# PKU-EPIC/GAPartNet

Hardware: AMD Instinct MI355X
Metric: point-clouds/sec (20k pts, train step) (higher is better)
Workload: dtype f32

## Files before the change

gapartnet_amd/_C.py:

```python
import ctypes
import os
import subprocess

_HERE = os.path.dirname(os.path.abspath(__file__))
SO_PATH = os.path.join(_HERE, "libgpn_hip.so")
CSRC = os.path.join(_HERE, "csrc")

_lib = None

_SIZE_T_FUNCS = (
    "gpn_voxelize_ws_bytes", "gpn_voxelize_scenes_ws_bytes", "gpn_rulebook_subm3_ws_bytes", "gpn_rulebook_down_ws_bytes",
    "gpn_rulebook_down_lists_ws_bytes", "gpn_rulebook_level_counts_ws_bytes", "gpn_spconv_fwd_ws_bytes", "gpn_spconv_fwd_w_ws_bytes", "gpn_net_ws_bytes", "gpn_linear_bwd_ws_bytes", "gpn_ball_query_grid_ws_bytes", "gpn_point_losses_ws_bytes", "gpn_rulebook_tile_order_ws_bytes", "gpn_bn_ws_bytes", "gpn_spconv_wgrad_ws_bytes", "gpn_ccl_ws_bytes", "gpn_nms_ws_bytes", "gpn_pn2_furthest_point_sampling_ws_bytes", "gpn_pose_fit_ws_bytes", "gpn_proposals_revoxelize_ws_bytes", "gpn_proposals_postprocess_ws_bytes", "gpn_backbone_prepare_arena_bytes", "gpn_scene_prepare_ws_bytes",
    "gpn_view_fps_ws_bytes", "gpn_net_forward_bf16_ws_bytes", "gpn_scene_maps_ws_bytes", "gpn_boxes_draw_ws_bytes",
    "gpn_pointmlp_wgrad_ws_bytes",
)


class GpnError(RuntimeError):
    pass


def build(jobs: int = 8) -> str:
    subprocess.check_call(["make", "-C", CSRC, "-s", "-j", str(jobs)])
    return SO_PATH


def lib():
    global _lib
    if _lib is None:
        if not os.path.exists(SO_PATH):
            raise GpnError(
                f"{SO_PATH} is missing: the HIP extension has not been built. Run "
                "`python -c 'import __graft_entry__ as g; g.build()'` (needs hipcc). There is no CPU fallback.")
        import torch
        _lib = ctypes.CDLL(SO_PATH)
        _lib.gpn_last_error.restype = ctypes.c_char_p
        _lib.gpn_entry_point_name.restype = ctypes.c_char_p
        for name in _SIZE_T_FUNCS:
            getattr(_lib, name).restype = ctypes.c_size_t
        vp, i64t, i32t, f32t, st = ctypes.c_void_p, ctypes.c_int64, ctypes.c_int, ctypes.c_float, ctypes.c_size_t
        _lib.gpn_spconv_fwd_w.argtypes = [vp, vp, i32t, i32t, i32t, i32t, vp, i64t, vp, vp, st, vp]
        _lib.gpn_spconv_wgrad.argtypes = [vp, vp, vp, vp, vp, i32t, i64t, i32t, i32t, i32t, vp, vp, st, vp]
        _lib.gpn_bn_fwd_train.argtypes = [vp, vp, vp, vp, i64t, i32t, f32t, f32t, i32t, vp, vp, vp, vp, vp, vp, st, vp]
        _lib.gpn_bn_fwd_eval.argtypes = [vp, vp, vp, vp, vp, vp, i64t, i32t, i32t, vp, vp]
        _lib.gpn_bn_bwd.argtypes = [vp, vp, vp, vp, vp, vp, i64t, i32t, i32t, i32t, vp, vp, vp, vp, vp, st, vp]
        _lib.gpn_gather_rows.argtypes = [vp, vp, i64t, i32t, vp, vp]
        _lib.gpn_scatter_rows_csr.argtypes = [vp, vp, vp, i64t, i32t, vp, vp]
        _lib.gpn_spconv_tiles_min_tiles.argtypes = [i64t]
        _lib.gpn_spconv_tiles_min_tiles.restype = i64t
        _lib.gpn_spconv_direct_split.argtypes = [i64t, i64t]
        _lib.gpn_spconv_msplit.argtypes = [i32t, i32t, i32t]
    return _lib


def check(rc: int, what: str = ""):
    if rc != 0:
        msg = lib().gpn_last_error().decode("utf-8", "replace")
        raise GpnError(f"{what or 'gpn call'} failed (code {rc}): {msg}")


def ptr(t):
    if t is None:
        return ctypes.c_void_p(0)
    return ctypes.c_void_p(t.data_ptr())


def i64(v):
    return ctypes.c_int64(int(v))


def i32(v):
    return ctypes.c_int(int(v))


def f32(v):
    return ctypes.c_float(float(v))


def szt(v):
    return ctypes.c_size_t(int(v))


def host_f32x3(v):
    return (ctypes.c_float * 3)(*[float(x) for x in v])


def host_i32x3(v):
    return (ctypes.c_int32 * 3)(*[int(x) for x in v])
```

gapartnet_amd/csrc/ballquery.hip:

```cpp
#include "gpn_common.h"

#include <rocprim/rocprim.hpp>

namespace {

constexpr int kThreads = 256;
constexpr int kWaves = kThreads / 64;
constexpr int kCap = 256;
constexpr int kMaxCell = 32766;

struct GridHeader {
  unsigned int min_enc[3];
  unsigned int overflow;
};

__device__ __forceinline__ unsigned int enc_float(float f) {
  const unsigned int b = __float_as_uint(f);
  return (b & 0x80000000u) ? ~b : (b | 0x80000000u);
}
__device__ __forceinline__ float dec_float(unsigned int u) {
  return __uint_as_float((u & 0x80000000u) ? (u & 0x7fffffffu) : ~u);
}

__global__ void bq_init_kernel(GridHeader* hdr) {
  hdr->min_enc[0] = hdr->min_enc[1] = hdr->min_enc[2] = 0xffffffffu;
  hdr->overflow = 0u;
}

__global__ __launch_bounds__(kThreads) void bq_min_kernel(const float* __restrict__ points, int64_t Np, GridHeader* hdr) {
  __shared__ unsigned int smin[3];
  if (threadIdx.x < 3) smin[threadIdx.x] = 0xffffffffu;
  __syncthreads();
  unsigned int m[3] = {0xffffffffu, 0xffffffffu, 0xffffffffu};
  for (int64_t j = (int64_t)blockIdx.x * kThreads + threadIdx.x; j < Np; j += (int64_t)gridDim.x * kThreads) {
#pragma unroll
    for (int a = 0; a < 3; ++a) {
      const unsigned int e = enc_float(points[j * 3 + a]);
      m[a] = e < m[a] ? e : m[a];
    }
  }
#pragma unroll
  for (int a = 0; a < 3; ++a) atomicMin(&smin[a], m[a]);
  __syncthreads();
  if (threadIdx.x < 3) atomicMin(&hdr->min_enc[threadIdx.x], smin[threadIdx.x]);
}

__device__ __forceinline__ int cell_of(float x, float origin, float inv_cell) {
  const float c = floorf(__fmul_rn(__fsub_rn(x, origin), inv_cell));
  return (int)fminf(fmaxf(c, -4.0f), 40000.0f) + 1;
}

__device__ __forceinline__ uint64_t pack_key(int seg, int cx, int cy, int cz) {
  return ((uint64_t)(unsigned)seg << 48) | ((uint64_t)(unsigned)cx << 32) | ((uint64_t)(unsigned)cy << 16) | (uint64_t)(unsigned)cz;
}

__global__ __launch_bounds__(kThreads) void bq_keys_kernel(const float* __restrict__ points,
                                                           const int32_t* __restrict__ point_labels,
                                                           const int32_t* __restrict__ batch_offsets, int64_t Np, int64_t S,
                                                           float inv_cell, GridHeader* hdr, uint64_t* __restrict__ keys,
                                                           int32_t* __restrict__ vals) {
  const int64_t j = (int64_t)blockIdx.x * kThreads + threadIdx.x;
  if (j >= Np) return;
  if (point_labels && point_labels[j] < 0) {
    keys[j] = ~0ull;
    vals[j] = (int32_t)j;
    return;
  }
  int64_t lo = 0, hi = S;
  while (hi - lo > 1) {
    const int64_t mid = (lo + hi) >> 1;
    if ((int64_t)batch_offsets[mid] <= j) lo = mid; else hi = mid;
  }
  const int seg = (int)lo;
  const float ox = dec_float(hdr->min_enc[0]), oy = dec_float(hdr->min_enc[1]), oz = dec_float(hdr->min_enc[2]);
  const int cx = cell_of(points[j * 3], ox, inv_cell), cy = cell_of(points[j * 3 + 1], oy, inv_cell),
            cz = cell_of(points[j * 3 + 2], oz, inv_cell);
  if (cx < 1 || cy < 1 || cz < 1 || cx > kMaxCell || cy > kMaxCell || cz > kMaxCell || seg > 65535) hdr->overflow = 1u;
  keys[j] = pack_key(seg & 0xffff, cx & 0x7fff, cy & 0x7fff, cz & 0x7fff);
  vals[j] = (int32_t)j;
}

__global__ __launch_bounds__(kThreads) void bq_records_kernel(const float* __restrict__ points,
                                                              const int32_t* __restrict__ point_labels,
                                                              const int32_t* __restrict__ order, int64_t Np,
                                                              float4* __restrict__ rec) {
  const int64_t j = (int64_t)blockIdx.x * kThreads + threadIdx.x;
  if (j >= Np) return;
  const int32_t o = order[j];
  float4 r;
  r.x = points[(int64_t)o * 3];
  r.y = points[(int64_t)o * 3 + 1];
  r.z = points[(int64_t)o * 3 + 2];
  r.w = __int_as_float(point_labels ? point_labels[o] : 0);
  rec[j] = r;
}

__device__ __forceinline__ bool is_hit(float qx, float qy, float qz, float px, float py, float pz, float r2) {
  const float dx = __fsub_rn(qx, px), dy = __fsub_rn(qy, py), dz = __fsub_rn(qz, pz);
  const float d2 = __fadd_rn(__fadd_rn(__fmul_rn(dx, dx), __fmul_rn(dy, dy)), __fmul_rn(dz, dz));
  return d2 < r2;
}

__global__ __launch_bounds__(kThreads) void bq_query_kernel(
    const float* __restrict__ points, const float* __restrict__ query, const int32_t* __restrict__ batch_indices,
    const int32_t* __restrict__ batch_offsets, const int32_t* __restrict__ point_labels,
    const int32_t* __restrict__ query_labels, int64_t Np, int64_t Q, float r2, float inv_cell, int K,
    const GridHeader* __restrict__ hdr, const uint64_t* __restrict__ keys, const int32_t* __restrict__ order,
    const float4* __restrict__ rec, int32_t* __restrict__ indices, int32_t* __restrict__ count) {
  __shared__ int32_t hits[kWaves][kCap];
  const int lane = threadIdx.x & 63, wave = threadIdx.x >> 6;
  const int64_t q = (int64_t)blockIdx.x * kWaves + wave;
  if (q >= Q) return;
  const float qx = query[q * 3], qy = query[q * 3 + 1], qz = query[q * 3 + 2];
  const int32_t b = batch_indices[q];
  const int32_t lo = batch_offsets[b], hi = batch_offsets[b + 1];
  const bool use_labels = point_labels != nullptr && query_labels != nullptr;
  const int32_t ql = use_labels ? query_labels[q] : 0;
  if (ql < 0) {
    if (lane == 0) count[q] = 0;
    return;
  }
  int32_t* out = indices + q * K;
  const uint64_t lane_lt = (1ull << lane) - 1ull;

  bool fallback = hdr->overflow != 0u || b > 65535;
  int H = 0;
  if (!fallback) {
    const float ox = dec_float(hdr->min_enc[0]), oy = dec_float(hdr->min_enc[1]), oz = dec_float(hdr->min_enc[2]);
    const int cx = cell_of(qx, ox, inv_cell), cy = cell_of(qy, oy, inv_cell), cz = cell_of(qz, oz, inv_cell);
    int32_t bound = 0;
    if (lane < 18) {
      const int t = lane < 9 ? lane : lane - 9;
      const int x = cx + t / 3 - 1, y = cy + t % 3 - 1;
      int z0 = cz - 1, z1 = cz + 1;
      const bool empty = x < 1 || y < 1 || x > kMaxCell || y > kMaxCell || z1 < 1 || z0 > kMaxCell;
      z0 = z0 < 1 ? 1 : z0;
      z1 = z1 > kMaxCell ? kMaxCell : z1;
      if (!empty) {
        const bool upper = lane >= 9;
        const uint64_t key = pack_key(b, x, y, upper ? z1 : z0);
        int64_t l = 0, h = Np;
        while (l < h) {
          const int64_t mid = (l + h) >> 1;
          const uint64_t k = keys[mid];
          if (upper ? (k <= key) : (k < key)) l = mid + 1; else h = mid;
        }
        bound = (int32_t)l;
      }
    }
    int32_t start[9], len[9];
    int total = 0;
#pragma unroll
    for (int t = 0; t < 9; ++t) {
      start[t] = __shfl(bound, t, 64);
      const int32_t e = __shfl(bound, t + 9, 64);
      len[t] = e > start[t] ? e - start[t] : 0;
      total += len[t];
    }
    for (int base = 0; base < total && !fallback; base += 64) {
      int c = base + lane;
      bool hit = false;
      int32_t o = -1;
      if (c < total) {
        int32_t j = 0;
#pragma unroll
        for (int t = 0; t < 9; ++t) {
          if (c >= 0 && c < len[t]) j = start[t] + c;
          c -= len[t];
        }
        const float4 r = rec[j];
        if (!use_labels || __float_as_int(r.w) == ql) {
          if (is_hit(qx, qy, qz, r.x, r.y, r.z, r2)) {
            o = order[j];
            hit = o >= lo && o < hi;
          }
        }
      }
      const uint64_t mask = __builtin_amdgcn_ballot_w64(hit);
      const int pos = H + __popcll(mask & lane_lt);
      if (hit && pos < kCap) hits[wave][pos] = o;
      H += __popcll(mask);
      if (H > kCap) fallback = true;
    }
  }

  if (!fallback) {
    for (int i = lane; i < H; i += 64) {
      const int32_t v = hits[wave][i];
      int rank = 0;
      for (int m = 0; m < H; ++m) rank += hits[wave][m] < v ? 1 : 0;
      if (rank < K) out[rank] = v;
    }
    if (lane == 0) count[q] = H < K ? H : K;
    return;
  }

  int cnt = 0;
  for (int32_t base = lo; base < hi && cnt < K; base += 64) {
    const int32_t j = base + lane;
    bool hit = false;
    if (j < hi && (!use_labels || point_labels[j] == ql))
      hit = is_hit(qx, qy, qz, points[(int64_t)j * 3], points[(int64_t)j * 3 + 1], points[(int64_t)j * 3 + 2], r2);
    const uint64_t mask = __builtin_amdgcn_ballot_w64(hit);
    const int pos = cnt + __popcll(mask & lane_lt);
    if (hit && pos < K) out[pos] = j;
    cnt += __popcll(mask);
  }
  if (lane == 0) count[q] = cnt < K ? cnt : K;
}

struct BqWs {
  GridHeader* hdr;
  uint64_t *keys, *keys_sorted;
  int32_t *vals, *order;
  float4* rec;
  void* prim_tmp;
  size_t prim_bytes, total;
};

BqWs carve(void* ws, size_t ws_bytes, int64_t Np) {
  gpn::WsCarver w(ws, ws_bytes);
  const size_t n = (size_t)(Np > 0 ? Np : 1);
  BqWs o;
  o.hdr = w.take<GridHeader>(1);
  o.keys = w.take<uint64_t>(n);
  o.keys_sorted = w.take<uint64_t>(n);
  o.vals = w.take<int32_t>(n);
  o.order = w.take<int32_t>(n);
  o.rec = w.take<float4>(n);
  o.prim_bytes = 0;
  (void)rocprim::radix_sort_pairs(nullptr, o.prim_bytes, (const uint64_t*)nullptr, (uint64_t*)nullptr,
                                  (const int32_t*)nullptr, (int32_t*)nullptr, n, 0, 64, (hipStream_t) nullptr);
  o.prim_tmp = w.take<char>(o.prim_bytes);
  o.total = w.used;
  return o;
}

}

extern "C" size_t gpn_ball_query_grid_ws_bytes(int64_t Np) { return carve(nullptr, 0, Np).total; }

extern "C" int gpn_ball_query_grid(const float* points, const float* query, const int32_t* batch_indices,
                                   const int32_t* batch_offsets, const int32_t* point_labels,
                                   const int32_t* query_labels, int64_t Np, int64_t Q, int64_t S, float radius, int K,
                                   int32_t* indices, int32_t* count, void* ws, size_t ws_bytes, gpn_stream_t stream_) {
  hipStream_t stream = (hipStream_t)stream_;
  const bool pad = !(K & GPN_BQ_NO_PAD);
  K &= ~GPN_BQ_NO_PAD;
  GPN_CHECK_ARG(Q >= 0 && Np >= 0 && S >= 0 && K >= 1 && radius > 0.f);
  if (Q == 0) return GPN_OK;
  GPN_CHECK_ARG(points && query && batch_indices && batch_offsets && indices && count);
  GPN_CHECK_ARG(Np < (int64_t)0x7fffffff && Q * (int64_t)K < ((int64_t)1 << 40));
  BqWs o = carve(ws, ws_bytes, Np);
  if (!ws || ws_bytes < o.total) {
    gpn::set_error("gpn_ball_query_grid: workspace too small (%zu needed, %zu given)", o.total, ws_bytes);
    return GPN_ERR_WS;
  }
  const float r2 = radius * radius;
  const float inv_cell = 1.0f / (1.05f * radius);
  gpn::ProfScope prof(GPN_K_BALL_QUERY, stream, 0.0, 12.0 * (double)Np + 4.0 * (double)Q * K);
  if (pad) GPN_CHECK_HIP(hipMemsetAsync(indices, 0xff, sizeof(int32_t) * (size_t)Q * K, stream));
  hipLaunchKernelGGL(bq_init_kernel, dim3(1), dim3(1), 0, stream, o.hdr);
  GPN_CHECK_LAUNCH();
  if (Np > 0) {
    const int pgrid = (int)gpn::cdiv(Np, kThreads);
    hipLaunchKernelGGL(bq_min_kernel, dim3(pgrid < 256 ? pgrid : 256), dim3(kThreads), 0, stream, points, Np, o.hdr);
    GPN_CHECK_LAUNCH();
    hipLaunchKernelGGL(bq_keys_kernel, dim3(pgrid), dim3(kThreads), 0, stream, points, point_labels, batch_offsets, Np, S,
                       inv_cell, o.hdr, o.keys, o.vals);
    GPN_CHECK_LAUNCH();
    size_t tmp = o.prim_bytes;
    GPN_CHECK_HIP(rocprim::radix_sort_pairs(o.prim_tmp, tmp, o.keys, o.keys_sorted, o.vals, o.order, (size_t)Np, 0, 64,
                                            stream));
    hipLaunchKernelGGL(bq_records_kernel, dim3(pgrid), dim3(kThreads), 0, stream, points, point_labels, o.order, Np,
                       o.rec);
    GPN_CHECK_LAUNCH();
  }
  hipLaunchKernelGGL(bq_query_kernel, dim3((unsigned)gpn::cdiv(Q, kWaves)), dim3(kThreads), 0, stream, points, query,
                     batch_indices, batch_offsets, point_labels, query_labels, Np, Q, r2, inv_cell, K, o.hdr,
                     o.keys_sorted, o.order, o.rec, indices, count);
  GPN_CHECK_LAUNCH();
  return GPN_OK;
}
```

gapartnet_amd/csrc/cluster.hip:

```cpp
#include "gpn_common.h"

namespace {

constexpr int kThreads = 256;

__global__ __launch_bounds__(kThreads) void ball_query_kernel(
    const float* __restrict__ points, const float* __restrict__ query, const int32_t* __restrict__ batch_indices,
    const int32_t* __restrict__ batch_offsets, const int32_t* __restrict__ point_labels,
    const int32_t* __restrict__ query_labels, int64_t Q, float r2, int K, int32_t* __restrict__ indices,
    int32_t* __restrict__ count) {
  __shared__ float4 tile[kThreads];
  __shared__ int32_t range_lo, range_hi;
  const int64_t q = (int64_t)blockIdx.x * kThreads + threadIdx.x;
  const bool active = q < Q;
  float qx = 0.f, qy = 0.f, qz = 0.f;
  int32_t lo = 0x7fffffff, hi = 0, ql = 0;
  if (active) {
    qx = query[q * 3]; qy = query[q * 3 + 1]; qz = query[q * 3 + 2];
    const int32_t b = batch_indices[q];
    lo = batch_offsets[b];
    hi = batch_offsets[b + 1];
    if (query_labels) ql = query_labels[q];
  }
  if (threadIdx.x == 0) { range_lo = 0x7fffffff; range_hi = 0; }
  __syncthreads();
  if (active && lo < hi) { atomicMin(&range_lo, lo); atomicMax(&range_hi, hi); }
  __syncthreads();
  const int32_t blo = range_lo, bhi = range_hi;
  const bool use_labels = point_labels != nullptr && query_labels != nullptr;
  int cnt = 0;
  int32_t* out = indices + q * K;
  for (int32_t base = blo; base < bhi; base += kThreads) {
    const int32_t j = base + threadIdx.x;
    if (j < bhi) {
      float4 rec;
      rec.x = points[(int64_t)j * 3]; rec.y = points[(int64_t)j * 3 + 1]; rec.z = points[(int64_t)j * 3 + 2];
      rec.w = __int_as_float(use_labels ? point_labels[j] : 0);
      tile[threadIdx.x] = rec;
    }
    __syncthreads();
    const int32_t n_here = (bhi - base < kThreads) ? (bhi - base) : kThreads;
    if (active && cnt < K && base < hi && base + n_here > lo) {
      int32_t t0 = lo > base ? lo - base : 0;
      int32_t t1 = hi - base < n_here ? hi - base : n_here;
      for (int32_t t = t0; t < t1 && cnt < K; ++t) {
        const float4 rec = tile[t];
        if (use_labels && __float_as_int(rec.w) != ql) continue;
        const float dx = __fsub_rn(qx, rec.x), dy = __fsub_rn(qy, rec.y), dz = __fsub_rn(qz, rec.z);
        const float d2 = __fadd_rn(__fadd_rn(__fmul_rn(dx, dx), __fmul_rn(dy, dy)), __fmul_rn(dz, dz));
        if (d2 < r2) out[cnt++] = base + t;
      }
    }
    const int done = (!active) || cnt >= K || (base + kThreads >= hi);
    if (__syncthreads_and(done)) break;
  }
  if (active) count[q] = cnt;
}

__device__ __forceinline__ int32_t uf_load(const int32_t* p) {
  return __hip_atomic_load(p, __ATOMIC_RELAXED, __HIP_MEMORY_SCOPE_WORKGROUP);
}
__device__ __forceinline__ int32_t uf_find(int32_t* parent, int32_t x) {
  int32_t p = uf_load(parent + x);
  while (p != x) {
    const int32_t gp = uf_load(parent + p);
    if (gp != p) __hip_atomic_store(parent + x, gp, __ATOMIC_RELAXED, __HIP_MEMORY_SCOPE_WORKGROUP);
    x = p;
    p = gp;
  }
  return x;
}
__device__ __forceinline__ void uf_union(int32_t* parent, int32_t ra, int32_t rb) {
  while (ra != rb) {
    if (ra < rb) { const int32_t tmp = ra; ra = rb; rb = tmp; }
    int32_t old = __hip_atomic_load(parent + ra, __ATOMIC_RELAXED, __HIP_MEMORY_SCOPE_AGENT);
    if (old == ra) {
      old = atomicCAS(parent + ra, ra, rb);
      if (old == ra) break;
    }
    ra = uf_find(parent, old);
    rb = uf_find(parent, rb);
  }
}

__global__ void ccl_init_kernel(const int32_t* __restrict__ begin_end, const int32_t* __restrict__ edges, int64_t Q,
                                int32_t* parent) {
  const int64_t v = ((int64_t)blockIdx.x * blockDim.x + threadIdx.x) >> 6;
  const int lane = threadIdx.x & 63;
  if (v >= Q) return;
  const int32_t b = begin_end[2 * v], e = begin_end[2 * v + 1];
  int32_t m = (int32_t)v;
  for (int32_t t = b + lane; t < e; t += 64) {
    const int32_t u = edges[t];
    if (u >= 0 && u < m) m = u;
  }
#pragma unroll
  for (int off = 32; off >= 1; off >>= 1) {
    const int32_t o = __shfl_xor(m, off, 64);
    m = o < m ? o : m;
  }
  if (lane == 0) parent[v] = m;
}

__global__ void ccl_compress_kernel(int32_t* parent, int64_t Q) {
  const int64_t i = (int64_t)blockIdx.x * blockDim.x + threadIdx.x;
  if (i >= Q) return;
  const int32_t r = uf_find(parent, (int32_t)i);
  if (r != (int32_t)i) __hip_atomic_store(parent + i, r, __ATOMIC_RELAXED, __HIP_MEMORY_SCOPE_WORKGROUP);
}

__global__ void ccl_hook_kernel(const int32_t* __restrict__ begin_end, const int32_t* __restrict__ edges,
                                int64_t Q, int32_t* parent) {
  const int64_t v = ((int64_t)blockIdx.x * blockDim.x + threadIdx.x) >> 6;
  const int lane = threadIdx.x & 63;
  if (v >= Q) return;
  const int32_t b = begin_end[2 * v], e = begin_end[2 * v + 1];
  for (int32_t t0 = b; t0 < e; t0 += 64) {
    const int32_t t = t0 + lane;
    int32_t u = t < e ? edges[t] : (int32_t)v;
    if (u < 0 || u >= Q) u = (int32_t)v;
    const int32_t pv = uf_load(parent + v);
    const bool same = uf_load(parent + u) == pv;
    if (__builtin_amdgcn_ballot_w64(!same) == 0) continue;
    const int32_t r = uf_find(parent, same ? (int32_t)v : u);
    int32_t m = r;
#pragma unroll
    for (int off = 32; off >= 1; off >>= 1) {
      const int32_t o = __shfl_xor(m, off, 64);
      m = o < m ? o : m;
    }
    uint64_t todo = __builtin_amdgcn_ballot_w64(r != m);
    while (todo) {
      const int leader = __builtin_ctzll(todo);
      const int32_t rl = __builtin_amdgcn_readlane(r, leader);
      if (lane == leader) uf_union(parent, rl, m);
      todo &= ~__builtin_amdgcn_ballot_w64(r == rl);
    }
  }
}

__global__ void ccl_flatten_kernel(int32_t* parent, int64_t Q, int32_t* __restrict__ labels,
                                   int32_t* __restrict__ is_root) {
  int64_t i = (int64_t)blockIdx.x * blockDim.x + threadIdx.x;
  if (i >= Q) return;
  const int32_t r = uf_find(parent, (int32_t)i);
  labels[i] = r;
  if (is_root) is_root[i] = (r == (int32_t)i) ? 1 : 0;
}

__global__ void ccl_rank_kernel(const int32_t* __restrict__ is_root, int64_t Q, int32_t* __restrict__ rank) {
  __shared__ int32_t sums[1024];
  __shared__ int32_t carry;
  if (threadIdx.x == 0) carry = 0;
  __syncthreads();
  for (int64_t base = 0; base < Q; base += 1024) {
    const int64_t i = base + threadIdx.x;
    const int32_t v = i < Q ? is_root[i] : 0;
    sums[threadIdx.x] = v;
    __syncthreads();
    for (int off = 1; off < 1024; off <<= 1) {
      int32_t t = threadIdx.x >= off ? sums[threadIdx.x - off] : 0;
      __syncthreads();
      sums[threadIdx.x] += t;
      __syncthreads();
    }
    if (i < Q) rank[i] = carry + sums[threadIdx.x] - v;
    __syncthreads();
    if (threadIdx.x == 1023) carry += sums[1023];
    __syncthreads();
  }
}
__global__ void ccl_relabel_kernel(int32_t* __restrict__ labels, const int32_t* __restrict__ rank, int64_t Q) {
  int64_t i = (int64_t)blockIdx.x * blockDim.x + threadIdx.x;
  if (i < Q) labels[i] = rank[labels[i]];
}

template <int MODE>
__global__ void segmented_reduce_kernel(const float* __restrict__ values, const int32_t* __restrict__ begin,
                                        const int32_t* __restrict__ end, int64_t P, int C,
                                        float* __restrict__ out) {
  int64_t t = (int64_t)blockIdx.x * blockDim.x + threadIdx.x;
  if (t >= P * C) return;
  const int64_t p = t / C;
  const int c = (int)(t - p * C);
  const int32_t b = begin[p], e = end[p];
  float acc = 0.f;
  for (int32_t r = b; r < e; ++r) {
    const float v = values[(int64_t)r * C + c];
    if (r == b) acc = v;
    else if (MODE == 0) acc = __fadd_rn(acc, v);
    else if (MODE == 1) acc = v < acc ? v : acc;
    else acc = v > acc ? v : acc;
  }
  out[t] = acc;
}

__global__ void segmented_maxpool_fwd_kernel(const float* __restrict__ values, const int32_t* __restrict__ begin,
                                             const int32_t* __restrict__ end, int64_t P, int C,
                                             float* __restrict__ pooled, int32_t* __restrict__ argmax) {
  int64_t t = (int64_t)blockIdx.x * blockDim.x + threadIdx.x;
  if (t >= P * C) return;
  const int64_t p = t / C;
  const int c = (int)(t - p * C);
  float best = 0.f;
  int32_t bi = -1;
  for (int32_t r = begin[p]; r < end[p]; ++r) {
    const float v = values[(int64_t)r * C + c];
    if (bi < 0 || v > best) { best = v; bi = r; }
  }
  pooled[t] = best;
  argmax[t] = bi;
}

__global__ __launch_bounds__(256) void segmented_maxpool_fwd_wg_kernel(const float* __restrict__ values,
                                                                       const int32_t* __restrict__ begin,
                                                                       const int32_t* __restrict__ end, int C,
                                                                       float* __restrict__ pooled, int32_t* __restrict__ argmax,
                                                                       int64_t P, const int64_t* __restrict__ p_dev) {
  __shared__ float sv[256];
  __shared__ int32_t si[256];
  P = gpn::live_rows(p_dev, P);
  const int R = 256 / C;
  const int c = threadIdx.x % C, rl = threadIdx.x / C;
  for (int64_t p = blockIdx.x; p < P; p += gridDim.x) {
  float best = 0.f;
  int32_t bi = -1;
  if (rl < R) {
    const int32_t b = begin[p], e = end[p];
    for (int32_t r = b + rl; r < e; r += R) {
      const float v = values[(int64_t)r * C + c];
      if (bi < 0 || v > best) { best = v; bi = r; }
    }
  }
  sv[threadIdx.x] = best;
  si[threadIdx.x] = bi;
  __syncthreads();
  if (threadIdx.x < C) {
    for (int q = 1; q < R; ++q) {
      const float v = sv[q * C + c];
      const int32_t i = si[q * C + c];
      if (i >= 0 && (bi < 0 || v > best || (v == best && i < bi))) { best = v; bi = i; }
    }
    pooled[p * C + c] = best;
    argmax[p * C + c] = bi;
  }
  __syncthreads();
  }
}

__global__ void segmented_maxpool_bwd_kernel(const float* __restrict__ dpooled, const int32_t* __restrict__ argmax,
                                             int64_t P, int C, float* __restrict__ dvalues, const int64_t* __restrict__ p_dev) {
  P = gpn::live_rows(p_dev, P);
  for (int64_t t = (int64_t)blockIdx.x * blockDim.x + threadIdx.x; t < P * C; t += (int64_t)gridDim.x * blockDim.x) {
    const int c = (int)(t % C);
    const int32_t r = argmax[t];
    if (r >= 0) dvalues[(int64_t)r * C + c] = dpooled[t];
  }
}
__global__ void zero_rows_kernel(float* __restrict__ p, int64_t rows, int C, const int64_t* __restrict__ m_dev) {
  const int64_t total = gpn::live_rows(m_dev, rows) * C;
  for (int64_t t = (int64_t)blockIdx.x * blockDim.x + threadIdx.x; t < total; t += (int64_t)gridDim.x * blockDim.x) p[t] = 0.f;
}

__global__ void instance_iou_kernel(const int32_t* __restrict__ proposal_offsets,
                                    const int32_t* __restrict__ instance_labels,
                                    const int32_t* __restrict__ batch_indices,
                                    const int32_t* __restrict__ npi, int64_t P, int I, float* __restrict__ ious,
                                    const int64_t* __restrict__ p_dev) {
  extern __shared__ int32_t hist[];
  P = gpn::live_rows(p_dev, P);
  for (int64_t p = blockIdx.x; p < P; p += gridDim.x) {
  const int32_t b0 = proposal_offsets[p], b1 = proposal_offsets[p + 1];
  for (int k = threadIdx.x; k < I; k += blockDim.x) hist[k] = 0;
  __syncthreads();
  for (int32_t m = b0 + threadIdx.x; m < b1; m += blockDim.x) {
    const int32_t l = instance_labels[m];
    if (l >= 0 && l < I) atomicAdd(&hist[l], 1);
  }
  __syncthreads();
  const int32_t b = b1 > b0 ? batch_indices[b0] : 0;
  for (int k = threadIdx.x; k < I; k += blockDim.x) {
    const int32_t n = npi[(int64_t)b * I + k];
    const int32_t uni = (b1 - b0) + n - hist[k];
    ious[p * I + k] = (n > 0 && uni > 0) ? __fdiv_rn((float)hist[k], (float)uni) : 0.f;
  }
  __syncthreads();
  }
}

__global__ void nms_mask_kernel(const float* __restrict__ ious, const int32_t* __restrict__ order, int64_t P,
                                int64_t W, float thr, unsigned long long* __restrict__ mask) {
  int64_t t = (int64_t)blockIdx.x * blockDim.x + threadIdx.x;
  if (t >= P * W) return;
  const int64_t a = t / W, w = t - a * W;
  const int32_t i = order[a];
  unsigned long long bits = 0;
  for (int bpos = 0; bpos < 64; ++bpos) {
    const int64_t bb = w * 64 + bpos;
    if (bb < P && bb > a && ious[(int64_t)i * P + order[bb]] > thr) bits |= 1ull << bpos;
  }
  mask[t] = bits;
}

__global__ void nms_scan_kernel(const unsigned long long* __restrict__ mask, const int32_t* __restrict__ order,
                                int64_t P, int64_t W, int32_t* __restrict__ keep, int32_t* __restrict__ num_keep) {
  extern __shared__ unsigned long long removed[];
  for (int64_t w = threadIdx.x; w < W; w += blockDim.x) removed[w] = 0;
  __syncthreads();
  int32_t n = 0;
  for (int64_t a = 0; a < P; ++a) {
    const bool dead = (removed[a >> 6] >> (a & 63)) & 1ull;
    __syncthreads();
    if (!dead) {
      if (threadIdx.x == 0) keep[n] = order[a];
      ++n;
      for (int64_t w = threadIdx.x; w < W; w += blockDim.x) removed[w] |= mask[a * W + w];
    }
    __syncthreads();
  }
  if (threadIdx.x == 0) num_keep[0] = n;
}

}

extern "C" int gpn_ball_query(const float* points, const float* query, const int32_t* batch_indices,
                              const int32_t* batch_offsets, const int32_t* point_labels,
                              const int32_t* query_labels, int64_t Np, int64_t Q, int64_t S, float radius, int K,
                              int32_t* indices, int32_t* count, gpn_stream_t stream_) {
  hipStream_t stream = (hipStream_t)stream_;
  GPN_CHECK_ARG(Q >= 0 && Np >= 0 && S >= 0 && K >= 1);
  if (Q == 0) return GPN_OK;
  GPN_CHECK_ARG(points && query && batch_indices && batch_offsets && indices && count);
  GPN_CHECK_ARG(Np < (int64_t)0x7fffffff);
  const float r2 = radius * radius;
  gpn::ProfScope prof(GPN_K_BALL_QUERY, stream, 0.0, 12.0 * (double)Np + 4.0 * (double)Q * K);
  GPN_CHECK_HIP(hipMemsetAsync(indices, 0xff, sizeof(int32_t) * (size_t)Q * K, stream));
  hipLaunchKernelGGL(ball_query_kernel, dim3((int)gpn::cdiv(Q, kThreads)), dim3(kThreads), 0, stream, points,
                     query, batch_indices, batch_offsets, point_labels, query_labels, Q, r2, K, indices, count);
  GPN_CHECK_LAUNCH();
  return GPN_OK;
}

extern "C" size_t gpn_ccl_ws_bytes(int64_t Q) {
  gpn::WsCarver w(nullptr, 0);
  size_t q = (size_t)(Q > 0 ? Q : 1);
  w.take<int32_t>(q);
  w.take<int32_t>(q);
  w.take<int32_t>(q);
  return w.used;
}

extern "C" int gpn_ccl(const int32_t* begin_end, const int32_t* edges, int64_t Q, int64_t E, int compacted,
                       int32_t* labels, void* ws, size_t ws_bytes, gpn_stream_t stream_) {
  hipStream_t stream = (hipStream_t)stream_;
  GPN_CHECK_ARG(Q >= 0 && E >= 0);
  if (Q == 0) return GPN_OK;
  GPN_CHECK_ARG(begin_end && labels && (edges || E == 0));
  GPN_CHECK_ARG(Q < (int64_t)0x7fffffff / 64);
  gpn::WsCarver w(ws, ws_bytes);
  int32_t* parent = w.take<int32_t>((size_t)Q);
  int32_t* is_root = w.take<int32_t>((size_t)Q);
  int32_t* rank = w.take<int32_t>((size_t)Q);
  GPN_CHECK_WS(w);
  const int grid = (int)gpn::cdiv(Q, kThreads);
  gpn::ProfScope prof(GPN_K_CCL, stream, 0.0, 4.0 * ((double)E + 2.0 * (double)Q) + 4.0 * (double)Q);
  hipLaunchKernelGGL(ccl_init_kernel, dim3((int)gpn::cdiv(Q * 64, kThreads)), dim3(kThreads), 0, stream, begin_end, edges,
                     Q, parent);
  GPN_CHECK_LAUNCH();
  hipLaunchKernelGGL(ccl_compress_kernel, dim3(grid), dim3(kThreads), 0, stream, parent, Q);
  GPN_CHECK_LAUNCH();
  hipLaunchKernelGGL(ccl_hook_kernel, dim3((int)gpn::cdiv(Q * 64, kThreads)), dim3(kThreads), 0, stream,
                     begin_end, edges, Q, parent);
  GPN_CHECK_LAUNCH();
  hipLaunchKernelGGL(ccl_flatten_kernel, dim3(grid), dim3(kThreads), 0, stream, parent, Q, labels,
                     compacted ? is_root : nullptr);
  GPN_CHECK_LAUNCH();
  if (compacted) {
    hipLaunchKernelGGL(ccl_rank_kernel, dim3(1), dim3(1024), 0, stream, is_root, Q, rank);
    GPN_CHECK_LAUNCH();
    hipLaunchKernelGGL(ccl_relabel_kernel, dim3(grid), dim3(kThreads), 0, stream, labels, rank, Q);
    GPN_CHECK_LAUNCH();
  }
  return GPN_OK;
}

extern "C" int gpn_segmented_reduce(const float* values, const int32_t* begin, const int32_t* end, int64_t P,
                                    int C, int mode, float* out, gpn_stream_t stream_) {
  hipStream_t stream = (hipStream_t)stream_;
  GPN_CHECK_ARG(P >= 0 && C >= 1 && mode >= 0 && mode <= 2);
  if (P == 0) return GPN_OK;
  GPN_CHECK_ARG(values && begin && end && out);
  const dim3 grid((int)gpn::cdiv(P * C, kThreads)), block(kThreads);
  if (mode == 0) hipLaunchKernelGGL(segmented_reduce_kernel<0>, grid, block, 0, stream, values, begin, end, P, C, out);
  else if (mode == 1) hipLaunchKernelGGL(segmented_reduce_kernel<1>, grid, block, 0, stream, values, begin, end, P, C, out);
  else hipLaunchKernelGGL(segmented_reduce_kernel<2>, grid, block, 0, stream, values, begin, end, P, C, out);
  GPN_CHECK_LAUNCH();
  return GPN_OK;
}

static int maxpool_fwd_impl(const float* values, const int32_t* begin, const int32_t* end, int64_t P, const gpn::DevRows& rows, int C,
                            float* pooled, int32_t* argmax, hipStream_t stream);
extern "C" int gpn_segmented_maxpool_fwd(const float* values, const int32_t* begin, const int32_t* end,
                                         int64_t P, int C, float* pooled, int32_t* argmax, gpn_stream_t stream_) {
  return maxpool_fwd_impl(values, begin, end, P, gpn::DevRows(), C, pooled, argmax, (hipStream_t)stream_);
}
extern "C" int gpn_segmented_maxpool_fwd_dev(const float* values, const int32_t* begin, const int32_t* end, int64_t P,
                                             const int64_t* p_dev, int64_t p_plan, int C, float* pooled, int32_t* argmax,
                                             gpn_stream_t stream_) {
  GPN_CHECK_ARG(p_dev != nullptr && C <= 256 && 256 % C == 0);
  return maxpool_fwd_impl(values, begin, end, P, gpn::DevRows{p_dev, p_plan}, C, pooled, argmax, (hipStream_t)stream_);
}
static int maxpool_fwd_impl(const float* values, const int32_t* begin, const int32_t* end, int64_t P, const gpn::DevRows& rows, int C,
                            float* pooled, int32_t* argmax, hipStream_t stream) {
  GPN_CHECK_ARG(P >= 0 && C >= 1);
  if (P == 0) return GPN_OK;
  GPN_CHECK_ARG(values && begin && end && pooled && argmax);
  if (C <= 256 && 256 % C == 0 && P < (int64_t)0x7fffffff)
    hipLaunchKernelGGL(segmented_maxpool_fwd_wg_kernel, dim3(gpn::dev_grid(P, gpn::plan_rows(P, rows), rows.dev != nullptr)), dim3(256), 0,
                       stream, values, begin, end, C, pooled, argmax, P, rows.dev);
  else
    hipLaunchKernelGGL(segmented_maxpool_fwd_kernel, dim3((int)gpn::cdiv(P * C, kThreads)), dim3(kThreads), 0,
                       stream, values, begin, end, P, C, pooled, argmax);
  GPN_CHECK_LAUNCH();
  return GPN_OK;
}

extern "C" int gpn_segmented_maxpool_bwd(const float* dpooled, const int32_t* argmax, int64_t P, int C,
                                         int64_t M, float* dvalues, gpn_stream_t stream_) {
  hipStream_t stream = (hipStream_t)stream_;
  GPN_CHECK_ARG(P >= 0 && C >= 1 && M >= 0);
  if (M > 0) {
    GPN_CHECK_ARG(dvalues);
    GPN_CHECK_HIP(hipMemsetAsync(dvalues, 0, sizeof(float) * (size_t)M * C, stream));
  }
  if (P == 0) return GPN_OK;
  GPN_CHECK_ARG(dpooled && argmax);
  hipLaunchKernelGGL(segmented_maxpool_bwd_kernel, dim3((int)gpn::cdiv(P * C, kThreads)), dim3(kThreads), 0,
                     stream, dpooled, argmax, P, C, dvalues, (const int64_t*)nullptr);
  GPN_CHECK_LAUNCH();
  return GPN_OK;
}
extern "C" int gpn_segmented_maxpool_bwd_dev(const float* dpooled, const int32_t* argmax, int64_t P, const int64_t* p_dev,
                                             int64_t p_plan, int C, int64_t M, const int64_t* m_dev, int64_t m_plan, float* dvalues,
                                             gpn_stream_t stream_) {
  hipStream_t stream = (hipStream_t)stream_;
  GPN_CHECK_ARG(P >= 1 && C >= 1 && M >= 1 && p_dev && m_dev && dpooled && argmax && dvalues);
  const int64_t mp = gpn::plan_rows(M, gpn::DevRows{m_dev, m_plan}), pp = gpn::plan_rows(P, gpn::DevRows{p_dev, p_plan});
  hipLaunchKernelGGL(zero_rows_kernel, dim3(gpn::dev_grid(gpn::cdiv(M * C, kThreads), gpn::cdiv(mp * C, kThreads), true)), dim3(kThreads), 0,
                     stream, dvalues, M, C, m_dev);
  GPN_CHECK_LAUNCH();
  hipLaunchKernelGGL(segmented_maxpool_bwd_kernel, dim3(gpn::dev_grid(gpn::cdiv(P * C, kThreads), gpn::cdiv(pp * C, kThreads), true)),
                     dim3(kThreads), 0, stream, dpooled, argmax, P, C, dvalues, p_dev);
  GPN_CHECK_LAUNCH();
  return GPN_OK;
}

static int instance_iou_impl(const int32_t* proposal_offsets, const int32_t* instance_labels, const int32_t* batch_indices,
                             const int32_t* num_points_per_instance, int64_t P, const gpn::DevRows& rows, int64_t B, int I, float* ious,
                             hipStream_t stream) {
  GPN_CHECK_ARG(P >= 0 && B >= 0 && I >= 0);
  if (P == 0 || I == 0) return GPN_OK;
  GPN_CHECK_ARG(proposal_offsets && instance_labels && batch_indices && num_points_per_instance && ious);
  GPN_CHECK_ARG(I <= 8192);
  hipLaunchKernelGGL(instance_iou_kernel, dim3(gpn::dev_grid(P, gpn::plan_rows(P, rows), rows.dev != nullptr)), dim3(128),
                     sizeof(int32_t) * I, stream, proposal_offsets, instance_labels, batch_indices, num_points_per_instance, P, I, ious,
                     rows.dev);
  GPN_CHECK_LAUNCH();
  return GPN_OK;
}
extern "C" int gpn_instance_iou(const int32_t* proposal_offsets, const int32_t* instance_labels,
                                const int32_t* batch_indices, const int32_t* num_points_per_instance, int64_t P,
                                int64_t B, int I, float* ious, gpn_stream_t stream_) {
  return instance_iou_impl(proposal_offsets, instance_labels, batch_indices, num_points_per_instance, P, gpn::DevRows(), B, I, ious,
                           (hipStream_t)stream_);
}
extern "C" int gpn_instance_iou_dev(const int32_t* proposal_offsets, const int32_t* instance_labels, const int32_t* batch_indices,
                                    const int32_t* num_points_per_instance, int64_t P, const int64_t* p_dev, int64_t p_plan, int64_t B,
                                    int I, float* ious, gpn_stream_t stream_) {
  GPN_CHECK_ARG(p_dev != nullptr);
  return instance_iou_impl(proposal_offsets, instance_labels, batch_indices, num_points_per_instance, P, gpn::DevRows{p_dev, p_plan}, B,
                           I, ious, (hipStream_t)stream_);
}

extern "C" size_t gpn_nms_ws_bytes(int64_t P) {
  int64_t W = gpn::cdiv(P > 0 ? P : 1, 64);
  return gpn::align_up((size_t)(P > 0 ? P : 1) * W * sizeof(unsigned long long));
}

extern "C" int gpn_nms(const float* ious, const int32_t* order, int64_t P, float threshold, int32_t* keep,
                       int32_t* num_keep, void* ws, size_t ws_bytes, gpn_stream_t stream_) {
  hipStream_t stream = (hipStream_t)stream_;
  GPN_CHECK_ARG(P >= 0 && num_keep);
  if (P == 0) {
    GPN_CHECK_HIP(hipMemsetAsync(num_keep, 0, sizeof(int32_t), stream));
    return GPN_OK;
  }
  GPN_CHECK_ARG(ious && order && keep);
  const int64_t W = gpn::cdiv(P, 64);
  GPN_CHECK_ARG(W * 8 <= 64 * 1024);
  if (!ws || ws_bytes < (size_t)P * W * sizeof(unsigned long long)) {
    gpn::set_error("gpn_nms: workspace too small");
    return GPN_ERR_WS;
  }
  unsigned long long* mask = static_cast<unsigned long long*>(ws);
  hipLaunchKernelGGL(nms_mask_kernel, dim3((int)gpn::cdiv(P * W, kThreads)), dim3(kThreads), 0, stream, ious,
                     order, P, W, threshold, mask);
  GPN_CHECK_LAUNCH();
  hipLaunchKernelGGL(nms_scan_kernel, dim3(1), dim3(64), sizeof(unsigned long long) * W, stream, mask, order, P,
                     W, keep, num_keep);
  GPN_CHECK_LAUNCH();
  return GPN_OK;
}
```

gapartnet_amd/csrc/gpn_common.h:

```cpp
#pragma once
#include <cstdlib>
#include <cstring>
#include <hip/hip_runtime.h>

#include <cstdint>
#include <cstdio>

#include "../../include/gpn.h"

namespace gpn {

void set_error(const char* fmt, ...);

struct ProfScope {
  int id;
  hipStream_t stream;
  hipEvent_t start = nullptr;
  int64_t tag = 0;
  ProfScope(int kernel_id, hipStream_t s, double flops, double bytes, int64_t tag = 0);
  ProfScope(int kernel_id, hipStream_t s, double flops, double bytes, const int64_t* rows_dev, int64_t bound, int64_t tag = 0);
  ~ProfScope();
};
inline int64_t prof_shape_tag(int K, int64_t n_dst, int cin, int cout, bool twin) {
  return ((int64_t)(twin ? 1 : 0) << 62) | ((int64_t)(K & 63) << 48) | ((int64_t)((cin / 16) & 255) << 40) |
         ((int64_t)((cout / 16) & 255) << 32) | (n_dst & 0xffffffffll);
}

struct DevRows {
  const int64_t* dev = nullptr;
  int64_t plan = 0;
};
inline int64_t plan_rows(int64_t n, const DevRows& r) {
  if (!r.dev || r.plan <= 0) return n;
  return r.plan < n ? r.plan : n;
}
__device__ __forceinline__ int64_t live_rows(const int64_t* dev, int64_t n) {
  if (!dev) return n;
  const int64_t v = __builtin_nontemporal_load(dev);
  return v < n ? (v > 0 ? v : 0) : n;
}
inline unsigned dev_grid(int64_t wgs_bound, int64_t wgs_plan, bool dev, int mult = 1, int64_t floor_wgs = 1024) {
  int64_t g = wgs_bound;
  if (dev) {
    int64_t want = wgs_plan + wgs_plan / 2 + mult;
    if (want < floor_wgs) want = floor_wgs;
    if (want < g) g = want;
  }
  if (g < 1) g = 1;
  g = (g + mult - 1) / mult * mult;
  return (unsigned)g;
}

constexpr int kMaxDevices = 64;

inline int64_t cdiv(int64_t a, int64_t b) { return (a + b - 1) / b; }

inline size_t align_up(size_t v, size_t a = 256) { return (v + a - 1) / a * a; }

struct WsCarver {
  char* base;
  size_t used = 0, cap;
  WsCarver(void* ws, size_t bytes) : base(static_cast<char*>(ws)), cap(bytes) {}
  template <typename T>
  T* take(size_t count) {
    size_t bytes = align_up(count * sizeof(T));
    T* p = reinterpret_cast<T*>(base + used);
    used += bytes;
    return p;
  }
  bool ok() const { return used <= cap && (base != nullptr || used == 0); }
};

constexpr int kStatSlots = 32;
inline int stat_slot_count(int64_t rows) {
  const int64_t tiles = (rows + 15) / 16;
  int s = 1;
  while (s < kStatSlots && tiles > 64 * (int64_t)s) s *= 2;
  return s;
}
struct ConvAffine {
  const float* mean = nullptr;
  const float* var = nullptr;
  const float* weight = nullptr;
  const float* bias = nullptr;
  const float* res = nullptr;
  float eps = 0.f;
  int relu = 0;
};
struct ConvTwin {
  const float* in = nullptr;
  const float* packed = nullptr;
  float* out = nullptr;
  unsigned long long* slab = nullptr;
  const float* x = nullptr;
  const float* y = nullptr;
  const float* mean = nullptr;
  const float* invstd = nullptr;
  ConvAffine ep;
};
struct ConvStats {
  unsigned long long* slab = nullptr;
  int slot_mask = kStatSlots - 1;
  const float* x = nullptr;
  const float* y = nullptr;
  const float* mean = nullptr;
  const float* invstd = nullptr;
  int relu = 0;
  ConvAffine ep;
  ConvTwin twin;
};
#ifdef __HIPCC__
struct AffineCol {
  float mu, is, w, b;
};
__device__ __forceinline__ AffineCol affine_col(const ConvAffine& ep, uint32_t col) {
  return AffineCol{ep.mean[col], 1.0f / sqrtf(ep.var[col] + ep.eps), ep.weight[col], ep.bias[col]};
}
__device__ __forceinline__ float affine_apply(const ConvAffine& ep, const AffineCol& c, float v, uint32_t e) {
  v = (v - c.mu) * c.is * c.w + c.b;
  if (ep.res) v += ep.res[e];
  if (ep.relu) v = v > 0.f ? v : 0.f;
  return v;
}
#endif
struct BnFwdPtrs {
  const float* x = nullptr;
  const float* res = nullptr;
  const void* partial = nullptr;
  const float* weight = nullptr;
  const float* bias = nullptr;
  float* y = nullptr;
  float* mean = nullptr;
  float* invstd = nullptr;
  float* running_mean = nullptr;
  float* running_var = nullptr;
};
struct BnBwdPtrs {
  const float* x = nullptr;
  const float* y = nullptr;
  const float* dy = nullptr;
  const void* partial = nullptr;
  const float* mean = nullptr;
  const float* invstd = nullptr;
  const float* weight = nullptr;
  float* dx = nullptr;
  float* dres = nullptr;
  float* dweight = nullptr;
  float* dbias = nullptr;
};
inline size_t stat_slab_bytes(int C) { return align_up((size_t)kStatSlots * 4 * C * sizeof(unsigned long long)); }

int spconv_fwd_into(const float* in, const float* packed_w, const int32_t* nbr, const int32_t* nbr_p, const int32_t* perm, int K,
                    int64_t n_dst, int cin, int cout, float* out, int accumulate, const ConvStats& stats, void* ws,
                    size_t ws_bytes, hipStream_t stream, const DevRows& rows = DevRows());
bool spconv_fwd_accumulates_stats(int K, int64_t n_dst, int cin, int cout);
bool spconv_fwd_accumulates_stats(int K, int64_t n_dst, int cin, int cout, const DevRows& rows);
bool spconv_fwd_applies_affine(int K, int64_t n_dst, int cin, int cout, const DevRows& rows);
bool spconv_tiles_supported(int K, int64_t n_dst, int cin, int cout);
int spconv_tiles_launch(const float* in, const float* packed, const int32_t* nbr, const int32_t* perm, int K, int64_t n_dst,
                        int cin, int cout, int accumulate, const ConvStats& stats, float* out, hipStream_t stream,
                        const DevRows& rows = DevRows());
bool spconv_msplit_supported(int K, int64_t n_dst, int cin, int cout);
int spconv_msplit_launch(const float* in, const float* packed, const int32_t* nbr, const int32_t* perm, int K, int64_t n_dst,
                         int cin, int cout, int accumulate, const ConvStats& stats, float* out, hipStream_t stream,
                         const DevRows& rows = DevRows());
struct PackBf16Desc {
  const float* W;
  uint16_t* packed;
  int K, cin, cout, oki;
};
int spconv_bf16_check(const char* who, int K, int64_t n_dst, int cin, int cout);
int spconv_bf16_launch(const uint16_t* in, const uint16_t* packed, const int32_t* nbr, const int32_t* nbr_p, const int32_t* perm,
                       int K, int64_t n_dst, int cin, int cout, const gpn_conv_epilogue_bf16_t* ep, void* out, hipStream_t stream);
int pack_bf16_many(const PackBf16Desc* descs, int n, hipStream_t stream);
int rows_to_bf16_launch(const float* x, int64_t total, uint16_t* y, hipStream_t stream);
int bn_act_bf16_launch(const void* x, int x_is_f32, const uint16_t* res, const float* weight, const float* bias, const float* mean,
                       const float* var, float eps, int64_t N, int C, int relu, int out_f32, void* y, hipStream_t stream);
int concat_bf16_launch(const uint16_t* a, const uint16_t* b, uint16_t* dst, int64_t rows, int ca, int cb, hipStream_t stream);
constexpr int kWgradReduceJobs = 24;
constexpr int kWgradSets = 4;
struct WgradSet {
  const float* in;
  const float* dout;
  const int32_t *pair_src, *pair_dst, *tile_off;
  float* partial;
};
struct WgradSets {
  int n = 0;
  WgradSet s[kWgradSets];
};
struct WgradReduceJob {
  const float* partial;
  float* dW;
  int64_t elems;
  int S, K, cin, cout, oki, few;
};
int wgrad_slices(int K, int cin, int cout, int64_t n_dst);
int wgrad_contract(const WgradSets& sets, int K, int64_t n_dst, int cin, int cout, int S, hipStream_t stream,
                   const int64_t* n_dst_dev = nullptr);
WgradReduceJob wgrad_reduce_job(const float* partial, int S, int K, int cin, int cout, int flags, float* dW);
int wgrad_reduce_many(const WgradReduceJob* jobs, int n, hipStream_t stream);
int rulebook_level_counts_dev(const int32_t* indices, int64_t n_max, const int64_t* n_dev, int64_t batch_size,
                              const int64_t* max_coord_dev, int n_levels, int64_t* counts, void* ws, size_t ws_bytes,
                              hipStream_t stream);
// ... 52 lines not shown
```

gapartnet_amd/csrc/gpn_core.hip:

```cpp
#include <cstdarg>
#include <algorithm>
#include <mutex>
#include <vector>

#include "gpn_common.h"

namespace {
thread_local char g_err[512] = "";

struct ProfRec {
  hipEvent_t a, b;
  int64_t tag;
};
struct ProfLive {
  const int64_t* rows_dev;
  int64_t bound;
  double flops, bytes;
};
struct ProfSlot {
  std::vector<ProfRec> recs;
  std::vector<ProfLive> live;
  double flops = 0, bytes = 0;
  int64_t launches = 0;
};
std::mutex g_prof_mu;
bool g_prof_on = false;
ProfSlot g_prof[GPN_K_COUNT];

const char* kEntryPoints[] = {
    "gpn_voxelize", "gpn_voxelize_ws_bytes", "gpn_rulebook_subm3", "gpn_rulebook_subm3_ws_bytes",
    "gpn_rulebook_down", "gpn_rulebook_down_ws_bytes", "gpn_rulebook_down_lists",
    "gpn_rulebook_down_lists_ws_bytes", "gpn_rulebook_level_counts", "gpn_rulebook_identity", "gpn_rulebook_level_counts_ws_bytes", "gpn_voxelize_ex", "gpn_voxelize_scenes", "gpn_voxelize_scenes_sorted", "gpn_voxelize_scenes_ws_bytes", "gpn_spconv_pack_weights", "gpn_spconv_fwd", "gpn_spconv_fwd_ws_bytes", "gpn_spconv_fwd_ordered", "gpn_rulebook_tile_order_ws_bytes", "gpn_rulebook_tile_order", "gpn_spconv_tiles_min_tiles", "gpn_spconv_direct_split", "gpn_spconv_msplit", "gpn_spconv_fwd_w", "gpn_spconv_fwd_w_ws_bytes", "gpn_spconv_wgrad",
    "gpn_spconv_wgrad_ws_bytes", "gpn_gather_rows", "gpn_scatter_rows_csr", "gpn_bn_ws_bytes", "gpn_bn_fwd_train", "gpn_bn_fwd_eval", "gpn_bn_bwd", "gpn_net_ws_bytes", "gpn_net_bn_fusion", "gpn_net_wgrad_group", "gpn_net_forward", "gpn_linear_supported", "gpn_linear_fwd", "gpn_linear_bwd_ws_bytes", "gpn_linear_bwd", "gpn_net_backward", "gpn_net_forward_pair", "gpn_net_backward_pair", "gpn_point_losses_ws_bytes", "gpn_point_losses_fwd", "gpn_point_losses_fwd_metrics", "gpn_point_losses_bwd", "gpn_score_loss", "gpn_npcs_loss_fwd", "gpn_npcs_loss_bwd", "gpn_ball_query", "gpn_ball_query_grid_ws_bytes", "gpn_ball_query_grid", "gpn_ccl",
    "gpn_ccl_ws_bytes", "gpn_segmented_reduce", "gpn_segmented_maxpool_fwd", "gpn_segmented_maxpool_bwd",
    "gpn_instance_iou", "gpn_nms", "gpn_nms_ws_bytes", "gpn_pn2_ball_query", "gpn_pn2_group_points",
    "gpn_pn2_group_points_grad", "gpn_pn2_gather_points", "gpn_pn2_gather_points_grad",
    "gpn_pn2_furthest_point_sampling", "gpn_pn2_furthest_point_sampling_ws_bytes",
    "gpn_pn2_furthest_point_sampling_ws", "gpn_pn2_three_nn", "gpn_pn2_knn", "gpn_pn2_three_interpolate",
    "gpn_pn2_three_interpolate_grad", "gpn_proposals_max_proposals", "gpn_proposals_build_ws_bytes", "gpn_proposals_build", "gpn_proposals_voxel_mean",
    "gpn_proposals_voxel_mean_bwd", "gpn_proposals_revoxelize_ws_bytes", "gpn_proposals_revoxelize", "gpn_proposals_postprocess_ws_bytes", "gpn_proposals_postprocess", "gpn_proposals_postprocess_lds_proposals", "gpn_backbone_prepare_desc_words", "gpn_backbone_prepare_arena_bytes", "gpn_backbone_prepare", "gpn_scene_prepare_max_instances", "gpn_scene_prepare_ws_bytes", "gpn_scene_prepare", "gpn_pose_fit_ws_bytes", "gpn_pose_fit", "gpn_copy_many", "gpn_adam_blocks", "gpn_adam_step", "gpn_adam_step_gated", "gpn_prof_enable", "gpn_prof_bracket_overhead_us", "gpn_prof_reset", "gpn_prof_get", "gpn_prof_get_launches",
    "gpn_rulebook_subm3_dev", "gpn_rulebook_down_dev_ws_bytes", "gpn_rulebook_down_dev", "gpn_rulebook_down_lists_dev", "gpn_rulebook_identity_dev", "gpn_gather_rows_dev", "gpn_scatter_rows_csr_dev", "gpn_proposals_voxel_mean_dev", "gpn_proposals_targets_dev", "gpn_linear_fwd_dev", "gpn_linear_bwd_dev", "gpn_segmented_maxpool_fwd_dev", "gpn_segmented_maxpool_bwd_dev", "gpn_instance_iou_dev", "gpn_score_loss_dev", "gpn_npcs_loss_fwd_dev", "gpn_npcs_loss_bwd_dev",
    "gpn_view_max_instance_ids", "gpn_view_backproject", "gpn_view_fps_ws_bytes", "gpn_view_fps", "gpn_view_finish",
    "gpn_spconv_pack_weights_bf16", "gpn_spconv_fwd_bf16", "gpn_rows_to_bf16", "gpn_bn_act_bf16", "gpn_net_forward_bf16_ws_bytes",
    "gpn_net_forward_bf16",
    "gpn_scene_maps_ws_bytes", "gpn_scene_maps", "gpn_points_winner", "gpn_points_paint", "gpn_boxes_draw_ws_bytes", "gpn_boxes_draw",
    "gpn_pointmlp_supported", "gpn_pointmlp_fwd", "gpn_pointmlp_wgrad_ws_bytes", "gpn_pointmlp_wgrad",
    "gpn_last_error", "gpn_version"};
}

namespace gpn {
void set_error(const char* fmt, ...) {
  va_list ap;
  va_start(ap, fmt);
  vsnprintf(g_err, sizeof(g_err), fmt, ap);
  va_end(ap);
}

ProfScope::ProfScope(int kernel_id, hipStream_t s, double flops, double bytes, int64_t tag_) : id(kernel_id), stream(s), tag(tag_) {
  if (!g_prof_on) return;
  std::lock_guard<std::mutex> lk(g_prof_mu);
  g_prof[id].flops += flops;
  g_prof[id].bytes += bytes;
  g_prof[id].launches += 1;
  if (hipEventCreate(&start) != hipSuccess) { start = nullptr; return; }
  hipEventRecord(start, stream);
}
ProfScope::ProfScope(int kernel_id, hipStream_t s, double flops, double bytes, const int64_t* rows_dev, int64_t bound, int64_t tag_)
    : ProfScope(kernel_id, s, rows_dev ? 0.0 : flops, rows_dev ? 0.0 : bytes, tag_) {
  if (!g_prof_on || !rows_dev) return;
  std::lock_guard<std::mutex> lk(g_prof_mu);
  g_prof[id].live.push_back({rows_dev, bound, flops, bytes});
}
ProfScope::~ProfScope() {
  if (!start) return;
  hipEvent_t stop;
  if (hipEventCreate(&stop) != hipSuccess) return;
  hipEventRecord(stop, stream);
  std::lock_guard<std::mutex> lk(g_prof_mu);
  g_prof[id].recs.push_back({start, stop, tag});
}
}

extern "C" {
const char* gpn_last_error(void) { return g_err; }
int gpn_version(void) { return 1; }
int gpn_num_entry_points(void) { return (int)(sizeof(kEntryPoints) / sizeof(kEntryPoints[0])); }
const char* gpn_entry_point_name(int i) {
  return (i >= 0 && i < gpn_num_entry_points()) ? kEntryPoints[i] : nullptr;
}

__global__ void gpn_prof_noop_kernel() {}

int gpn_prof_bracket_overhead_us(gpn_stream_t stream_, double* overhead_us) {
  hipStream_t stream = (hipStream_t)stream_;
  GPN_CHECK_ARG(overhead_us != nullptr);
  constexpr int kReps = 33;
  hipEvent_t a[kReps], b[kReps];
  for (int i = 0; i < kReps; ++i) {
    GPN_CHECK_HIP(hipEventCreate(&a[i]));
    GPN_CHECK_HIP(hipEventCreate(&b[i]));
  }
  for (int i = 0; i < kReps; ++i) {
    GPN_CHECK_HIP(hipEventRecord(a[i], stream));
    hipLaunchKernelGGL(gpn_prof_noop_kernel, dim3(1), dim3(64), 0, stream);
    GPN_CHECK_HIP(hipEventRecord(b[i], stream));
  }
  GPN_CHECK_HIP(hipEventSynchronize(b[kReps - 1]));
  float t[kReps];
  for (int i = 0; i < kReps; ++i) {
    GPN_CHECK_HIP(hipEventElapsedTime(&t[i], a[i], b[i]));
    hipEventDestroy(a[i]);
    hipEventDestroy(b[i]);
  }
  std::sort(t, t + kReps);
  *overhead_us = (double)t[kReps / 2] * 1e3;
  return GPN_OK;
}

int gpn_prof_enable(int on) {
  std::lock_guard<std::mutex> lk(g_prof_mu);
  g_prof_on = on != 0;
  return GPN_OK;
}
int gpn_prof_reset(void) {
  std::lock_guard<std::mutex> lk(g_prof_mu);
  for (auto& s : g_prof) {
    for (auto& r : s.recs) { hipEventDestroy(r.a); hipEventDestroy(r.b); }
    s.recs.clear();
    s.live.clear();
    s.flops = s.bytes = 0;
    s.launches = 0;
  }
  return GPN_OK;
}
int gpn_prof_get(int kernel_id, int64_t* launches_host, double* ms_host, double* flops_host,
                 double* bytes_host) {
  GPN_CHECK_ARG(kernel_id >= 0 && kernel_id < GPN_K_COUNT);
  std::lock_guard<std::mutex> lk(g_prof_mu);
  ProfSlot& s = g_prof[kernel_id];
  double ms = 0;
  for (auto& r : s.recs) {
    GPN_CHECK_HIP(hipEventSynchronize(r.b));
    float t = 0;
    GPN_CHECK_HIP(hipEventElapsedTime(&t, r.a, r.b));
    ms += t;
  }
  double live_flops = 0, live_bytes = 0;
  for (auto& l : s.live) {
    int64_t n = 0;
    GPN_CHECK_HIP(hipMemcpy(&n, l.rows_dev, sizeof(n), hipMemcpyDeviceToHost));
    n = n < 0 ? 0 : (n > l.bound ? l.bound : n);
    const double share = l.bound > 0 ? (double)n / (double)l.bound : 0.0;
    live_flops += l.flops * share;
    live_bytes += l.bytes * share;
  }
  if (launches_host) *launches_host = s.launches;
  if (ms_host) *ms_host = ms;
  if (flops_host) *flops_host = s.flops + live_flops;
  if (bytes_host) *bytes_host = s.bytes + live_bytes;
  return GPN_OK;
}
int gpn_prof_get_launches(int kernel_id, int64_t cap, double* ms_host, int64_t* tag_host, int64_t* count_host) {
  GPN_CHECK_ARG(kernel_id >= 0 && kernel_id < GPN_K_COUNT && cap >= 0 && count_host && (cap == 0 || (ms_host && tag_host)));
  std::lock_guard<std::mutex> lk(g_prof_mu);
  ProfSlot& s = g_prof[kernel_id];
  int64_t i = 0;
  for (auto& r : s.recs) {
    if (i < cap) {
      GPN_CHECK_HIP(hipEventSynchronize(r.b));
      float t = 0;
      GPN_CHECK_HIP(hipEventElapsedTime(&t, r.a, r.b));
      ms_host[i] = t;
      tag_host[i] = r.tag;
    }
    ++i;
  }
  *count_host = i;
  return GPN_OK;
}
}
```

gapartnet_amd/csrc/proposals.hip:

```cpp
#include "gpn_common.h"

#include <mutex>
#include <rocprim/rocprim.hpp>

namespace {

constexpr int kThreads = 256;

enum { kQ = 0, kM = 1, kP = 2, kV = 3, kDropped = 4, kRuns = 5, kCoarse = 6, kCounts = 8 };

__global__ __launch_bounds__(kThreads) void prop_label_kernel(const float* __restrict__ points, int stride,
                                                              const float* __restrict__ offsets,
                                                              const int64_t* __restrict__ sem_preds,
                                                              const int32_t* __restrict__ inst, int64_t N,
                                                              int32_t* __restrict__ lab, int32_t* __restrict__ flag,
                                                              uint8_t* __restrict__ valid_mask, float* __restrict__ xyz,
                                                              float* __restrict__ xyz_shift) {
  const int64_t i = (int64_t)blockIdx.x * kThreads + threadIdx.x;
  if (i >= N) return;
  const int64_t s = sem_preds[i];
  const bool ok = s > 0 && (inst == nullptr || inst[i] >= 0);
  lab[i] = ok ? (int32_t)s : -1;
  flag[i] = ok ? 1 : 0;
  valid_mask[i] = ok ? 1 : 0;
#pragma unroll
  for (int a = 0; a < 3; ++a) {
    const float p = points[i * stride + a];
    xyz[i * 3 + a] = p;
    xyz_shift[i * 3 + a] = __fadd_rn(p, offsets[i * 3 + a]);
  }
}

__global__ __launch_bounds__(kThreads) void prop_valid_kernel(const int32_t* __restrict__ flag,
                                                              const int32_t* __restrict__ rank, int64_t N,
                                                              int64_t* __restrict__ valid_indices, int64_t* __restrict__ counts) {
  const int64_t i = (int64_t)blockIdx.x * kThreads + threadIdx.x;
  if (i >= N) return;
  if (flag[i]) valid_indices[rank[i]] = i;
  if (i == N - 1) counts[kQ] = (int64_t)rank[i] + flag[i];
}

__global__ void prop_scene_offsets_kernel(const int32_t* __restrict__ batch_indices, int64_t N, int64_t B,
                                          int32_t* __restrict__ scene_off) {
  const int64_t b = (int64_t)blockIdx.x * blockDim.x + threadIdx.x;
  if (b > B) return;
  int64_t lo = 0, hi = N;
  while (lo < hi) {
    const int64_t mid = (lo + hi) >> 1;
    if ((int64_t)batch_indices[mid] < b) lo = mid + 1; else hi = mid;
  }
  scene_off[b] = (int32_t)lo;
}

__global__ __launch_bounds__(kThreads) void prop_begin_end_kernel(const int32_t* __restrict__ count, int64_t N, int K,
                                                                  int32_t* __restrict__ begin_end) {
  const int64_t i = (int64_t)blockIdx.x * kThreads + threadIdx.x;
  if (i >= N) return;
  begin_end[2 * i] = (int32_t)(i * K);
  begin_end[2 * i + 1] = (int32_t)(i * K) + count[i];
}

__global__ __launch_bounds__(kThreads) void prop_keys_kernel(const int32_t* __restrict__ lab, const int32_t* __restrict__ la,
                                                             const int32_t* __restrict__ lb, int64_t N,
                                                             uint32_t* __restrict__ keys, uint32_t* __restrict__ vals) {
  const int64_t c = (int64_t)blockIdx.x * kThreads + threadIdx.x;
  if (c >= 2 * N) return;
  const int64_t i = c < N ? c : c - N;
  uint32_t k = (uint32_t)(2 * N);
  if (lab[i] >= 0) k = c < N ? (uint32_t)la[i] : (uint32_t)(N + lb[i]);
  keys[c] = k;
  vals[c] = (uint32_t)c;
}

__global__ __launch_bounds__(kThreads) void prop_run_flags_kernel(const uint32_t* __restrict__ skeys, int64_t T2,
                                                                  uint32_t invalid, int32_t* __restrict__ start) {
  const int64_t i = (int64_t)blockIdx.x * kThreads + threadIdx.x;
  if (i >= T2) return;
  const uint32_t k = skeys[i];
  start[i] = (k != invalid && (i == 0 || skeys[i - 1] != k)) ? 1 : 0;
}

__global__ __launch_bounds__(kThreads) void prop_run_pos_kernel(const int32_t* __restrict__ start,
                                                                const int32_t* __restrict__ incl, int64_t T2,
                                                                int32_t* __restrict__ run_pos, int64_t* __restrict__ counts) {
  const int64_t i = (int64_t)blockIdx.x * kThreads + threadIdx.x;
  if (i >= T2) return;
  if (start[i]) run_pos[incl[i] - 1] = (int32_t)i;
  if (i == T2 - 1) counts[kRuns] = incl[i];
}

__global__ __launch_bounds__(kThreads) void prop_run_keep_kernel(const int32_t* __restrict__ run_pos,
                                                                 const int64_t* __restrict__ counts, int64_t T2,
                                                                 int min_points, int32_t* __restrict__ run_size,
                                                                 int32_t* __restrict__ keep_run) {
  const int64_t r = (int64_t)blockIdx.x * kThreads + threadIdx.x;
  if (r >= T2) return;
  const int64_t R = counts[kRuns], active = 2 * counts[kQ];
  int32_t size = 0;
  if (r < R) size = (int32_t)((r + 1 < R ? (int64_t)run_pos[r + 1] : active) - run_pos[r]);
  run_size[r] = size;
  keep_run[r] = size >= min_points ? 1 : 0;
}

__global__ __launch_bounds__(kThreads) void prop_elem_keep_kernel(const uint32_t* __restrict__ skeys,
                                                                  const int32_t* __restrict__ incl,
                                                                  const int32_t* __restrict__ keep_run, int64_t T2,
                                                                  uint32_t invalid, int32_t* __restrict__ keep_elem) {
  const int64_t i = (int64_t)blockIdx.x * kThreads + threadIdx.x;
  if (i >= T2) return;
  keep_elem[i] = (skeys[i] != invalid && keep_run[incl[i] - 1]) ? 1 : 0;
}

struct ScatterOut {
  int64_t *sorted_indices, *point_indices, *proposal_indices, *sizes;
  int32_t *batch_p, *sem_p, *inst_p, *proposal_offsets, *member_slot;
  float* xyz_p;
  int64_t* seg64;
};

__global__ __launch_bounds__(kThreads) void prop_scatter_kernel(
    const uint32_t* __restrict__ svals, const int32_t* __restrict__ start, const int32_t* __restrict__ incl,
    const int32_t* __restrict__ keep_elem, const int32_t* __restrict__ slot, const int32_t* __restrict__ run_size,
    const int32_t* __restrict__ new_pid, const int32_t* __restrict__ rank, const int32_t* __restrict__ lab,
    const int32_t* __restrict__ inst, const int32_t* __restrict__ batch_indices, const float* __restrict__ xyz, int64_t N,
    int64_t T2, ScatterOut o, int64_t* __restrict__ counts) {
  const int64_t i = (int64_t)blockIdx.x * kThreads + threadIdx.x;
  if (i >= T2) return;
  if (i == T2 - 1) counts[kM] = (int64_t)slot[i] + keep_elem[i];
  if (!keep_elem[i]) return;
  const int32_t run = incl[i] - 1;
  const int32_t p = new_pid[run];
  const int64_t m = slot[i];
  const uint32_t c = svals[i];
  const int64_t pt = c < (uint32_t)N ? c : c - (uint32_t)N;
  o.sorted_indices[m] = rank[pt];
  o.point_indices[m] = pt;
  o.proposal_indices[m] = p;
  o.batch_p[m] = batch_indices[pt];
  o.sem_p[m] = lab[pt];
  o.inst_p[m] = inst ? inst[pt] : 0;
  o.xyz_p[m * 3] = xyz[pt * 3], o.xyz_p[m * 3 + 1] = xyz[pt * 3 + 1], o.xyz_p[m * 3 + 2] = xyz[pt * 3 + 2];
  o.member_slot[c] = (int32_t)m;
  if (start[i]) {
    o.sizes[p] = run_size[run];
    o.proposal_offsets[p] = (int32_t)m;
  }
}

__global__ __launch_bounds__(kThreads) void prop_close_kernel(const int32_t* __restrict__ keep_run,
                                                              const int32_t* __restrict__ new_pid, int64_t T2, int64_t P_ub,
                                                              int32_t* __restrict__ proposal_offsets,
                                                              int64_t* __restrict__ seg64, int64_t* __restrict__ counts) {
  const int64_t p = (int64_t)blockIdx.x * kThreads + threadIdx.x;
  if (p > P_ub) return;
  const int64_t P = (int64_t)new_pid[T2 - 1] + keep_run[T2 - 1];
  const int64_t M = counts[kM];
  if (p == 0) counts[kP] = P;
  if (p >= P) proposal_offsets[p] = (int32_t)M;
  seg64[p] = p < P ? (int64_t)proposal_offsets[p] : M;
}

__global__ __launch_bounds__(kThreads) void prop_stats_kernel(const float* __restrict__ xyz_p,
                                                              const int32_t* __restrict__ proposal_offsets,
                                                              const int64_t* __restrict__ counts, const float* __restrict__ jitter,
                                                              float full, float inv_full, float max_scale,
                                                              float* __restrict__ mean_out,
                                                              float* __restrict__ scale_out, float* __restrict__ shift_out) {
  __shared__ float buf[kThreads / 64][64 * 3];
  const int lane = threadIdx.x & 63, wave = threadIdx.x >> 6;
  const int64_t p = (int64_t)blockIdx.x * (kThreads / 64) + wave;
  if (p >= counts[kP]) return;
  const int32_t b = proposal_offsets[p], e = proposal_offsets[p + 1];
  float* sb = buf[wave];
  float acc = 0.f;
  for (int32_t base = b; base < e; base += 64) {
    const int32_t n = e - base < 64 ? e - base : 64;
    for (int t = lane; t < n * 3; t += 64) sb[t] = xyz_p[(int64_t)base * 3 + t];
    __builtin_amdgcn_wave_barrier();
    __builtin_amdgcn_s_waitcnt(0);
    if (lane < 3)
      for (int j = 0; j < n; ++j) acc = __fadd_rn(acc, sb[j * 3 + lane]);
    __builtin_amdgcn_wave_barrier();
  }
  const float cnt = (float)(e - b);
  const float mean_l = __fdiv_rn(acc, cnt);
  const float m0 = __shfl(mean_l, 0, 64), m1 = __shfl(mean_l, 1, 64), m2 = __shfl(mean_l, 2, 64);
  float lo[3] = {INFINITY, INFINITY, INFINITY}, hi[3] = {-INFINITY, -INFINITY, -INFINITY};
  const float mu[3] = {m0, m1, m2};
  for (int32_t j = b + lane; j < e; j += 64) {
#pragma unroll
    for (int a = 0; a < 3; ++a) {
// ... 191 lines not shown
  int total;
  int run = revox_thread_scan(s, wave_tot, total);
  for (int i = b; i < e; ++i) {
    const int c = a[i];
    a[i] = run;
    run += c;
  }
  __syncthreads();
  return total;
}

__global__ __launch_bounds__(kThreads) void revox_place_kernel(const float* __restrict__ scaled,
                                                               const int32_t* __restrict__ proposal_offsets,
                                                               const int64_t* __restrict__ counts, float full, int D, int64_t T2,
                                                               const int32_t* __restrict__ vox_base, const int32_t* __restrict__ kept_base,
                                                               const int32_t* __restrict__ out_base, int32_t* __restrict__ vc3,
                                                               int32_t* __restrict__ vseg, int32_t* __restrict__ pc_voxel_id,
                                                               int32_t* __restrict__ point_order, int32_t* __restrict__ vstart) {
  __shared__ int cur[kRevoxMaxCells + 1];
  __shared__ uint32_t bm[kRevoxWords];
  __shared__ int wprefix[kRevoxWords];
  __shared__ int wave_tot[4];
  const int t = threadIdx.x, lane = t & 63, wave = t >> 6;
  const int cells = D * D * D, words = (cells + 31) >> 5;
  const int64_t P = counts[kP], T = counts[kM];
  const int kept_total = kept_base[P];
  auto local_voxel = [&](int cell) {
    const uint32_t word = bm[cell >> 5];
    return wprefix[cell >> 5] + __builtin_popcount(word & ((1u << (cell & 31)) - 1u));
  };
  for (int64_t p = blockIdx.x; p < P; p += gridDim.x) {
    for (int w = t; w < words; w += kThreads) bm[w] = 0u;
    __syncthreads();
    const int64_t b = proposal_offsets[p], e = proposal_offsets[p + 1];
    for (int64_t m = b + t; m < e; m += kThreads) {
      const int cell = revox_cell(scaled, m, full, D);
      if (cell >= 0) atomicOr(&bm[cell >> 5], 1u << (cell & 31));
    }
    __syncthreads();
    for (int w = t; w < words; w += kThreads) wprefix[w] = __builtin_popcount(bm[w]);
    __syncthreads();
    const int n_vox = revox_block_scan(wprefix, words, wave_tot);
    for (int v = t; v <= n_vox; v += kThreads) cur[v] = 0;
    __syncthreads();
    for (int64_t m = b + t; m < e; m += kThreads) {
      const int cell = revox_cell(scaled, m, full, D);
      atomicAdd(&cur[cell >= 0 ? local_voxel(cell) : n_vox], 1);
    }
    __syncthreads();
    revox_block_scan(cur, n_vox, wave_tot);
    if (t == 0) cur[n_vox] = 0;
    const int vb = vox_base[p], kb = kept_base[p], ob = kept_total + out_base[p];
    for (int w = t; w < words; w += kThreads) {
      uint32_t word = bm[w];
      int vid = vb + wprefix[w];
      while (word) {
        const int bit = __builtin_ctz(word);
        word &= word - 1u;
        const int c = w * 32 + bit;
        vstart[vid] = kb + cur[vid - vb];
        vc3[(int64_t)vid * 3 + 2] = c % D;
        vc3[(int64_t)vid * 3 + 1] = (c / D) % D;
        vc3[(int64_t)vid * 3 + 0] = c / (D * D);
        vseg[vid] = (int32_t)p;
        ++vid;
      }
    }
    __syncthreads();
    for (int64_t m0 = b; m0 < e; m0 += kThreads) {
      const int64_t m = m0 + t;
      int key = -1;
      if (m < e) {
        const int cell = revox_cell(scaled, m, full, D);
        key = cell >= 0 ? local_voxel(cell) : n_vox;
      }
      uint64_t same = __builtin_amdgcn_ballot_w64(key >= 0);
#pragma unroll
      for (int bit = 0; bit < 16; ++bit) {
        const uint64_t has = __builtin_amdgcn_ballot_w64(((key >> bit) & 1) != 0);
        same &= ((key >> bit) & 1) ? has : ~has;
      }
      const int earlier = __builtin_popcountll(same & ((1ull << lane) - 1ull));
      const int group = __builtin_popcountll(same);
      for (int wv = 0; wv < 4; ++wv) {
        if (wave == wv && key >= 0) {
          const int base = cur[key];
          const int pos = (key < n_vox ? kb : ob) + base + earlier;
          point_order[pos] = (int32_t)m;
          pc_voxel_id[m] = key < n_vox ? vb + key : -1;
          if (earlier == 0) cur[key] = base + group;
        }
        __syncthreads();
      }
    }
  }
  for (int64_t m = T + (int64_t)blockIdx.x * kThreads + t; m < T2; m += (int64_t)gridDim.x * kThreads) {
    point_order[m] = (int32_t)m;
    pc_voxel_id[m] = -1;
  }
}

__global__ __launch_bounds__(kThreads) void prop_voxel_mean_kernel(const float* __restrict__ feats,
                                                                   const int64_t* __restrict__ point_indices,
                                                                   const int32_t* __restrict__ order,
                                                                   const int32_t* __restrict__ vstart, int64_t V, int C,
                                                                   float* __restrict__ out, const int64_t* __restrict__ v_dev) {
  V = gpn::live_rows(v_dev, V);
  for (int64_t t = (int64_t)blockIdx.x * kThreads + threadIdx.x; t < V * C; t += (int64_t)gridDim.x * kThreads) {
    const int64_t v = t / C;
    const int c = (int)(t - v * C);
    const int32_t b = vstart[v], e = vstart[v + 1];
    float acc = 0.f;
    for (int32_t j = b; j < e; ++j) acc = __fadd_rn(acc, feats[point_indices[order[j]] * C + c]);
    out[v * C + c] = __fdiv_rn(acc, (float)(e - b));
  }
}

__global__ __launch_bounds__(kThreads) void prop_targets_kernel(const int64_t* __restrict__ sem_labels, const float* __restrict__ gt_npcs,
                                                                const int64_t* __restrict__ point_indices, int64_t M,
                                                                const int64_t* __restrict__ m_dev, int64_t* __restrict__ sem_out,
                                                                float* __restrict__ npcs_out) {
  M = gpn::live_rows(m_dev, M);
  for (int64_t m = (int64_t)blockIdx.x * kThreads + threadIdx.x; m < M; m += (int64_t)gridDim.x * kThreads) {
    const int64_t i = point_indices[m];
    if (sem_labels) sem_out[m] = sem_labels[i];
    if (gt_npcs) {
      npcs_out[m * 3] = gt_npcs[i * 3], npcs_out[m * 3 + 1] = gt_npcs[i * 3 + 1], npcs_out[m * 3 + 2] = gt_npcs[i * 3 + 2];
    }
  }
}

__global__ __launch_bounds__(kThreads) void prop_voxel_mean_bwd_kernel(const float* __restrict__ dout,
                                                                       const int32_t* __restrict__ member_slot,
                                                                       const int32_t* __restrict__ pc_voxel_id,
                                                                       const int32_t* __restrict__ vstart, int64_t N, int C,
                                                                       float* __restrict__ dfeats) {
  const int64_t t = (int64_t)blockIdx.x * kThreads + threadIdx.x;
  const int64_t i = t / C;
  const int c = (int)(t - i * C);
  if (i >= N) return;
  float g = 0.f;
#pragma unroll
  for (int set = 0; set < 2; ++set) {
    const int32_t m = member_slot[set * N + i];
    if (m < 0) continue;
    const int32_t v = pc_voxel_id[m];
    if (v < 0) continue;
    g = __fadd_rn(g, __fdiv_rn(dout[(int64_t)v * C + c], (float)(vstart[v + 1] - vstart[v])));
  }
  dfeats[i * C + c] = g;
}

struct PropWs {
  int32_t *lab, *flag, *rank, *scene_off, *cnt, *begin_end, *la, *lb, *start, *incl, *run_pos, *run_size, *keep_run, *new_pid,
      *keep_elem, *slot, *vc3, *vseg, *nbr, *rv_nvox, *rv_nout, *rv_vbase, *rv_kbase, *rv_obase;
  uint32_t *keys, *skeys, *vals, *svals;
  float *xyz, *xyz_shift, *mean, *scale, *shift, *scaled, *rmin, *rmax, *vf;
  int64_t* seg64;
  void *prim, *sub;
  size_t prim_bytes, sub_bytes, total;
};

size_t prim_bytes_for(int64_t T2) {
  size_t a = 0, b = 0, c = 0;
  const size_t n = (size_t)(T2 > 0 ? T2 : 1);
  (void)rocprim::radix_sort_pairs(nullptr, a, (const uint32_t*)nullptr, (uint32_t*)nullptr, (const uint32_t*)nullptr,
                                  (uint32_t*)nullptr, n, 0u, 32u, (hipStream_t) nullptr);
  (void)rocprim::inclusive_scan(nullptr, b, (const int32_t*)nullptr, (int32_t*)nullptr, n, rocprim::plus<int32_t>(),
                                (hipStream_t) nullptr);
  (void)rocprim::exclusive_scan(nullptr, c, (const int32_t*)nullptr, (int32_t*)nullptr, 0, n, rocprim::plus<int32_t>(),
                                (hipStream_t) nullptr);
  return std::max(a, std::max(b, c));
}

PropWs carve(void* ws, size_t ws_bytes, int64_t N, int64_t B, int Kmax, int64_t P_ub) {
  gpn::WsCarver w(ws, ws_bytes);
  const size_t n = (size_t)(N > 0 ? N : 1), t2 = 2 * n, pu = (size_t)P_ub + 1;
  PropWs o;
  o.lab = w.take<int32_t>(n), o.flag = w.take<int32_t>(n), o.rank = w.take<int32_t>(n);
  o.scene_off = w.take<int32_t>((size_t)B + 2);
  o.cnt = w.take<int32_t>(n), o.begin_end = w.take<int32_t>(2 * n), o.la = w.take<int32_t>(n), o.lb = w.take<int32_t>(n);
  o.start = w.take<int32_t>(t2), o.incl = w.take<int32_t>(t2), o.run_pos = w.take<int32_t>(t2), o.run_size = w.take<int32_t>(t2);
  o.keep_run = w.take<int32_t>(t2), o.new_pid = w.take<int32_t>(t2), o.keep_elem = w.take<int32_t>(t2), o.slot = w.take<int32_t>(t2);
  o.vc3 = w.take<int32_t>(3 * t2), o.vseg = w.take<int32_t>(t2);
  o.keys = w.take<uint32_t>(t2), o.skeys = w.take<uint32_t>(t2), o.vals = w.take<uint32_t>(t2), o.svals = w.take<uint32_t>(t2);
  o.xyz = w.take<float>(3 * n), o.xyz_shift = w.take<float>(3 * n);
  o.mean = w.take<float>(3 * pu), o.scale = w.take<float>(pu), o.shift = w.take<float>(3 * pu);
  o.scaled = w.take<float>(3 * t2), o.rmin = w.take<float>(3 * pu), o.rmax = w.take<float>(3 * pu), o.vf = w.take<float>(3 * t2);
  o.seg64 = w.take<int64_t>(pu);
  o.rv_nvox = w.take<int32_t>(pu + 1), o.rv_nout = w.take<int32_t>(pu + 1), o.rv_vbase = w.take<int32_t>(pu + 1);
  o.rv_kbase = w.take<int32_t>(pu + 1), o.rv_obase = w.take<int32_t>(pu + 1);
  o.nbr = w.take<int32_t>(n * (size_t)Kmax);
  o.prim_bytes = prim_bytes_for((int64_t)t2);
  o.prim = w.take<char>(o.prim_bytes);
  o.sub_bytes = std::max(std::max(gpn_ball_query_grid_ws_bytes(N), gpn_ccl_ws_bytes(N)), gpn_voxelize_ws_bytes((int64_t)t2, 3));
  o.sub_bytes = std::max(o.sub_bytes, gpn_rulebook_level_counts_ws_bytes((int64_t)t2, 1));
  o.sub = w.take<char>(o.sub_bytes);
  o.total = w.used;
  return o;
}

inline int grid_of(int64_t n) { return (int)gpn::cdiv(n > 0 ? n : 1, kThreads); }

bool revox_fits(float fullscale) {
  const int64_t D = (int64_t)fullscale + 1;
  return fullscale >= 1.0f && D * D * D <= kRevoxMaxCells;
}
int revoxelize(const float* scaled, const int32_t* proposal_offsets, int64_t* counts, int64_t T2, int64_t P_ub, float fullscale,
               int32_t* vc3, int32_t* vseg, int32_t* pc_voxel_id, int32_t* point_order, int32_t* vstart, int32_t* n_vox,
               int32_t* n_out, int32_t* vox_base, int32_t* kept_base, int32_t* out_base, hipStream_t stream) {
  const int D = (int)fullscale + 1;
  const int64_t pw = P_ub > 0 ? P_ub : 1;
  hipLaunchKernelGGL(revox_count_kernel, dim3((unsigned)std::min<int64_t>(pw, 2048)), dim3(kThreads), 0, stream, scaled,
                     proposal_offsets, counts, fullscale, D, n_vox, n_out);
  GPN_CHECK_LAUNCH();
  hipLaunchKernelGGL(revox_scan_kernel, dim3(1), dim3(1024), 0, stream, proposal_offsets, counts, n_vox, n_out, vox_base, kept_base,
                     out_base, vstart);
  GPN_CHECK_LAUNCH();
  hipLaunchKernelGGL(revox_place_kernel, dim3((unsigned)std::min<int64_t>(std::max<int64_t>(pw, 256), 512)), dim3(kThreads), 0, stream,
                     scaled, proposal_offsets, counts, fullscale, D, T2, vox_base, kept_base, out_base, vc3, vseg, pc_voxel_id,
                     point_order, vstart);
  GPN_CHECK_LAUNCH();
  return GPN_OK;
}

}

extern "C" int64_t gpn_proposals_max_proposals(int64_t N, int min_points) {
  return 2 * N / (min_points > 0 ? min_points : 1) + 1;
}

extern "C" size_t gpn_proposals_build_ws_bytes(int64_t N, int64_t B, int K1, int K2, int min_points) {
  return carve(nullptr, 0, N, B, K1 > K2 ? K1 : K2, gpn_proposals_max_proposals(N, min_points)).total;
}

extern "C" int gpn_proposals_build(const float* points, int point_stride, const float* offset_preds, const int64_t* sem_preds,
                                   const int32_t* instance_labels, const int32_t* batch_indices, int64_t N, int64_t B,
                                   float radius, int K1, int K2, int min_points, float fullscale, float max_scale,
                                   const float* jitter, int64_t* counts, uint8_t* valid_mask, int64_t* valid_indices,
                                   int64_t* sorted_indices, int64_t* point_indices, int64_t* proposal_indices,
                                   int32_t* batch_indices_p, float* pt_xyz_p, int32_t* sem_preds_p, int32_t* instance_labels_p,
                                   int64_t* sizes, int32_t* proposal_offsets, int32_t* member_slot, int32_t* voxel_coords4,
                                   int32_t* pc_voxel_id, int32_t* point_order, int32_t* voxel_point_start, void* ws,
                                   size_t ws_bytes, gpn_stream_t stream_) {
  hipStream_t stream = (hipStream_t)stream_;
  GPN_CHECK_ARG(N >= 1 && B >= 1 && K1 >= 1 && K2 >= 1 && min_points >= 1 && point_stride >= 3 && radius > 0.f);
  GPN_CHECK_ARG(N < ((int64_t)1 << 30) && (int64_t)N * (K1 > K2 ? K1 : K2) < ((int64_t)1 << 31));
  GPN_CHECK_ARG(points && offset_preds && sem_preds && batch_indices && jitter && counts && valid_mask && valid_indices);
  GPN_CHECK_ARG(sorted_indices && point_indices && proposal_indices && batch_indices_p && pt_xyz_p && sem_preds_p);
  GPN_CHECK_ARG(instance_labels_p && sizes && proposal_offsets && member_slot && voxel_coords4 && pc_voxel_id);
  GPN_CHECK_ARG(point_order && voxel_point_start);
  const int64_t P_ub = gpn_proposals_max_proposals(N, min_points);
  const int64_t T2 = 2 * N;
  PropWs o = carve(ws, ws_bytes, N, B, K1 > K2 ? K1 : K2, P_ub);
  if (!ws || ws_bytes < o.total) {
    gpn::set_error("gpn_proposals_build: workspace too small (%zu needed, %zu given)", o.total, ws_bytes);
    return GPN_ERR_WS;
  }
  GPN_CHECK_HIP(hipMemsetAsync(counts, 0, sizeof(int64_t) * kCounts, stream));
  GPN_CHECK_HIP(hipMemsetAsync(member_slot, 0xff, sizeof(int32_t) * (size_t)T2, stream));

  hipLaunchKernelGGL(prop_label_kernel, dim3(grid_of(N)), dim3(kThreads), 0, stream, points, point_stride, offset_preds,
                     sem_preds, instance_labels, N, o.lab, o.flag, valid_mask, o.xyz, o.xyz_shift);
  GPN_CHECK_LAUNCH();
  size_t tmp = o.prim_bytes;
  GPN_CHECK_HIP(rocprim::exclusive_scan(o.prim, tmp, o.flag, o.rank, 0, (size_t)N, rocprim::plus<int32_t>(), stream));
  hipLaunchKernelGGL(prop_valid_kernel, dim3(grid_of(N)), dim3(kThreads), 0, stream, o.flag, o.rank, N, valid_indices, counts);
  GPN_CHECK_LAUNCH();
  hipLaunchKernelGGL(prop_scene_offsets_kernel, dim3((int)gpn::cdiv(B + 1, 64)), dim3(64), 0, stream, batch_indices, N, B,
                     o.scene_off);
  GPN_CHECK_LAUNCH();

  const float* coords[2] = {o.xyz, o.xyz_shift};
  const int ks[2] = {K1, K2};
  int32_t* labels[2] = {o.la, o.lb};
  for (int set = 0; set < 2; ++set) {
    hipStream_t st = stream;
    int32_t *nbr = o.nbr, *cnt = o.cnt, *begin_end = o.begin_end;
    void* sub = o.sub;
    const size_t sub_bytes = o.sub_bytes;
    int rc = gpn_ball_query_grid(coords[set], coords[set], batch_indices, o.scene_off, o.lab, o.lab, N, N, B, radius,
                                 ks[set] | GPN_BQ_NO_PAD, nbr, cnt, sub, sub_bytes, (gpn_stream_t)st);
    if (rc) return rc;
    hipLaunchKernelGGL(prop_begin_end_kernel, dim3(grid_of(N)), dim3(kThreads), 0, st, cnt, N, ks[set], begin_end);
    GPN_CHECK_LAUNCH();
    rc = gpn_ccl(begin_end, nbr, N, N * (int64_t)ks[set], 0, labels[set], sub, sub_bytes, (gpn_stream_t)st);
    if (rc) return rc;
  }
  hipLaunchKernelGGL(prop_keys_kernel, dim3(grid_of(T2)), dim3(kThreads), 0, stream, o.lab, o.la, o.lb, N, o.keys, o.vals);
  GPN_CHECK_LAUNCH();
  unsigned bits = 1;
  while (bits < 32 && ((uint64_t)T2 >> bits) != 0) ++bits;
  tmp = o.prim_bytes;
  GPN_CHECK_HIP(rocprim::radix_sort_pairs(o.prim, tmp, o.keys, o.skeys, o.vals, o.svals, (size_t)T2, 0u, bits, stream));

  const uint32_t invalid = (uint32_t)T2;
  hipLaunchKernelGGL(prop_run_flags_kernel, dim3(grid_of(T2)), dim3(kThreads), 0, stream, o.skeys, T2, invalid, o.start);
  GPN_CHECK_LAUNCH();
  tmp = o.prim_bytes;
  GPN_CHECK_HIP(rocprim::inclusive_scan(o.prim, tmp, o.start, o.incl, (size_t)T2, rocprim::plus<int32_t>(), stream));
  hipLaunchKernelGGL(prop_run_pos_kernel, dim3(grid_of(T2)), dim3(kThreads), 0, stream, o.start, o.incl, T2, o.run_pos, counts);
  GPN_CHECK_LAUNCH();
  hipLaunchKernelGGL(prop_run_keep_kernel, dim3(grid_of(T2)), dim3(kThreads), 0, stream, o.run_pos, counts, T2, min_points,
                     o.run_size, o.keep_run);
  GPN_CHECK_LAUNCH();
  tmp = o.prim_bytes;
  GPN_CHECK_HIP(rocprim::exclusive_scan(o.prim, tmp, o.keep_run, o.new_pid, 0, (size_t)T2, rocprim::plus<int32_t>(), stream));
  hipLaunchKernelGGL(prop_elem_keep_kernel, dim3(grid_of(T2)), dim3(kThreads), 0, stream, o.skeys, o.incl, o.keep_run, T2,
                     invalid, o.keep_elem);
  GPN_CHECK_LAUNCH();
  tmp = o.prim_bytes;
  GPN_CHECK_HIP(rocprim::exclusive_scan(o.prim, tmp, o.keep_elem, o.slot, 0, (size_t)T2, rocprim::plus<int32_t>(), stream));
  ScatterOut so{sorted_indices, point_indices, proposal_indices, sizes, batch_indices_p, sem_preds_p, instance_labels_p,
                proposal_offsets, member_slot, pt_xyz_p, o.seg64};
  hipLaunchKernelGGL(prop_scatter_kernel, dim3(grid_of(T2)), dim3(kThreads), 0, stream, o.svals, o.start, o.incl, o.keep_elem,
                     o.slot, o.run_size, o.new_pid, o.rank, o.lab, instance_labels, batch_indices, o.xyz, N, T2, so, counts);
  GPN_CHECK_LAUNCH();
  hipLaunchKernelGGL(prop_close_kernel, dim3(grid_of(P_ub + 1)), dim3(kThreads), 0, stream, o.keep_run, o.new_pid, T2, P_ub,
                     proposal_offsets, o.seg64, counts);
  GPN_CHECK_LAUNCH();

  hipLaunchKernelGGL(prop_stats_kernel, dim3((int)gpn::cdiv(P_ub, kThreads / 64)), dim3(kThreads), 0, stream, pt_xyz_p,
                     proposal_offsets, counts, jitter, fullscale, 1.0f / fullscale, max_scale, o.mean, o.scale, o.shift);
  GPN_CHECK_LAUNCH();
  hipLaunchKernelGGL(prop_scale_points_kernel, dim3(grid_of(T2)), dim3(kThreads), 0, stream, pt_xyz_p, proposal_indices, counts,
                     o.mean, o.scale, o.shift, T2, o.scaled);
  GPN_CHECK_LAUNCH();
  if (revox_fits(fullscale)) {
    int rc = revoxelize(o.scaled, proposal_offsets, counts, T2, P_ub, fullscale, o.vc3, o.vseg, pc_voxel_id, point_order,
                        voxel_point_start, o.rv_nvox, o.rv_nout, o.rv_vbase, o.rv_kbase, o.rv_obase, stream);
    if (rc) return rc;
  } else {
    hipLaunchKernelGGL(prop_ranges_kernel, dim3(grid_of(P_ub * 3)), dim3(kThreads), 0, stream, P_ub, fullscale, o.rmin, o.rmax);
    GPN_CHECK_LAUNCH();
    const float vs[3] = {1.0f, 1.0f, 1.0f};
    const int32_t dims[3] = {(int32_t)fullscale + 1, (int32_t)fullscale + 1, (int32_t)fullscale + 1};
    int rc = gpn_voxelize_ex(o.scaled, o.scaled, o.seg64, o.rmin, o.rmax, T2, 3, P_ub, vs, dims, o.vf, o.vc3, o.vseg, pc_voxel_id,
                             counts + kV, point_order, voxel_point_start, o.sub, o.sub_bytes, stream_);
    if (rc) return rc;
  }
  hipLaunchKernelGGL(prop_finish_kernel, dim3(grid_of(T2)), dim3(kThreads), 0, stream, o.vc3, o.vseg, pc_voxel_id, T2,
                     voxel_coords4, counts);
  GPN_CHECK_LAUNCH();
  const int32_t grid_shape[3] = {(int32_t)fullscale, (int32_t)fullscale, (int32_t)fullscale};
  return gpn_rulebook_level_counts(voxel_coords4, T2, counts + kV, P_ub > 0 ? P_ub : 1, grid_shape, 1, counts + kCoarse, o.sub, o.sub_bytes,
                                   stream_);
}

static int voxel_mean_impl(const float* feats, const int64_t* point_indices, const int32_t* point_order,
                           const int32_t* voxel_point_start, int64_t V, const gpn::DevRows& rows, int C, float* out, hipStream_t stream) {
  GPN_CHECK_ARG(V >= 0 && C >= 1);
  if (V == 0) return GPN_OK;
  GPN_CHECK_ARG(feats && point_indices && point_order && voxel_point_start && out);
  hipLaunchKernelGGL(prop_voxel_mean_kernel,
                     dim3(gpn::dev_grid(gpn::cdiv(V * C, kThreads), gpn::cdiv(gpn::plan_rows(V, rows) * C, kThreads), rows.dev != nullptr)),
                     dim3(kThreads), 0, stream, feats, point_indices, point_order, voxel_point_start, V, C, out, rows.dev);
  GPN_CHECK_LAUNCH();
  return GPN_OK;
}

extern "C" int gpn_proposals_voxel_mean(const float* feats, const int64_t* point_indices, const int32_t* point_order,
                                        const int32_t* voxel_point_start, int64_t V, int C, float* out, gpn_stream_t stream_) {
  return voxel_mean_impl(feats, point_indices, point_order, voxel_point_start, V, gpn::DevRows(), C, out, (hipStream_t)stream_);
}
extern "C" int gpn_proposals_voxel_mean_dev(const float* feats, const int64_t* point_indices, const int32_t* point_order,
                                            const int32_t* voxel_point_start, int64_t V, const int64_t* v_dev, int64_t v_plan, int C,
                                            float* out, gpn_stream_t stream_) {
  GPN_CHECK_ARG(v_dev != nullptr);
  return voxel_mean_impl(feats, point_indices, point_order, voxel_point_start, V, gpn::DevRows{v_dev, v_plan}, C, out,
                         (hipStream_t)stream_);
}
extern "C" int gpn_proposals_targets_dev(const int64_t* sem_labels, const float* gt_npcs, const int64_t* point_indices, int64_t M,
                                         const int64_t* m_dev, int64_t m_plan, int64_t* sem_out, float* npcs_out, gpn_stream_t stream_) {
  hipStream_t stream = (hipStream_t)stream_;
  GPN_CHECK_ARG(M >= 1 && m_dev && point_indices && (!sem_labels || sem_out) && (!gt_npcs || npcs_out));
  hipLaunchKernelGGL(prop_targets_kernel,
                     dim3(gpn::dev_grid(gpn::cdiv(M, kThreads), gpn::cdiv(gpn::plan_rows(M, gpn::DevRows{m_dev, m_plan}), kThreads), true)),
                     dim3(kThreads), 0, stream, sem_labels, gt_npcs, point_indices, M, m_dev, sem_out, npcs_out);
  GPN_CHECK_LAUNCH();
  return GPN_OK;
}

extern "C" int gpn_proposals_voxel_mean_bwd(const float* dout, const int32_t* member_slot, const int32_t* pc_voxel_id,
                                            const int32_t* voxel_point_start, int64_t N, int C, float* dfeats,
                                            gpn_stream_t stream_) {
  hipStream_t stream = (hipStream_t)stream_;
  GPN_CHECK_ARG(N >= 0 && C >= 1);
  if (N == 0) return GPN_OK;
  GPN_CHECK_ARG(dout && member_slot && pc_voxel_id && voxel_point_start && dfeats);
  hipLaunchKernelGGL(prop_voxel_mean_bwd_kernel, dim3(grid_of(N * C)), dim3(kThreads), 0, stream, dout, member_slot,
                     pc_voxel_id, voxel_point_start, N, C, dfeats);
  GPN_CHECK_LAUNCH();
  return GPN_OK;
}

extern "C" size_t gpn_proposals_revoxelize_ws_bytes(int64_t P_ub) {
  gpn::WsCarver w(nullptr, 0);
  for (int k = 0; k < 5; ++k) w.take<int32_t>((size_t)(P_ub > 0 ? P_ub : 1) + 2);
  return w.used;
}
extern "C" int gpn_proposals_revoxelize(const float* scaled, const int32_t* proposal_offsets, int64_t* counts, int64_t T2, int64_t P_ub,
                                        float fullscale, int32_t* voxel_coords3, int32_t* voxel_seg, int32_t* pc_voxel_id,
                                        int32_t* point_order, int32_t* voxel_point_start, void* ws, size_t ws_bytes,
                                        gpn_stream_t stream_) {
  GPN_CHECK_ARG(T2 >= 1 && P_ub >= 1 && scaled && proposal_offsets && counts);
  GPN_CHECK_ARG(voxel_coords3 && voxel_seg && pc_voxel_id && point_order && voxel_point_start);
  if (!revox_fits(fullscale)) {
    gpn::set_error("gpn_proposals_revoxelize: a grid of (%d + 1)^3 cells does not fit one workgroup's LDS (max %d cells)", (int)fullscale,
                   kRevoxMaxCells);
    return GPN_ERR_ARG;
  }
  gpn::WsCarver w(ws, ws_bytes);
  int32_t* a[5];
  for (int k = 0; k < 5; ++k) a[k] = w.take<int32_t>((size_t)P_ub + 2);
  GPN_CHECK_WS(w);
  return revoxelize(scaled, proposal_offsets, counts, T2, P_ub, fullscale, voxel_coords3, voxel_seg, pc_voxel_id, point_order,
                    voxel_point_start, a[0], a[1], a[2], a[3], a[4], (hipStream_t)stream_);
}
```

gapartnet_amd/hip_ops.py:

```python
from dataclasses import dataclass
from typing import Optional

import numpy as np
import torch

from . import _C
from ._C import check, f32, host_f32x3, host_i32x3, i32, i64, ptr, szt

TILE_ROWS = 32
PACK_TRANSPOSE = 1
PACK_REVERSE = 2
name = "hip"


def _stream():
    return _C.ctypes.c_void_p(torch._C._cuda_getCurrentRawStream(torch.cuda.current_device()))


def _dev(*tensors):
    dev = None
    for t in tensors:
        if t is None:
            continue
        if not t.is_cuda:
# ... 539 lines not shown


def point_losses_fwd(logits, labels, offsets, gt_offsets, instance_labels, ignore_index, metrics=False):
    dev = _dev(logits, offsets)
    logits, offsets, gt_offsets = _c(logits, torch.float32), _c(offsets, torch.float32), _c(gt_offsets, torch.float32)
    labels, instance_labels = _c(labels, torch.int64), _c(instance_labels, torch.int32)
    M, C = logits.shape
    losses = torch.empty((4,), dtype=torch.float32, device=dev)
    stats = torch.empty((4,), dtype=torch.float64, device=dev)
    L = _C.lib()
    ws = _ws(L.gpn_point_losses_ws_bytes(i64(M)), dev)
    if metrics:
        preds = torch.empty((M,), dtype=torch.int64, device=dev)
        accu = torch.empty((2,), dtype=torch.float32, device=dev)
        check(L.gpn_point_losses_fwd_metrics(ptr(logits), ptr(labels), ptr(offsets), ptr(gt_offsets), ptr(instance_labels), i64(M),
                                             i32(C), i64(ignore_index), ptr(losses), ptr(preds), ptr(accu), ptr(stats), ptr(ws),
                                             szt(ws.numel()), _stream()), "gpn_point_losses_fwd_metrics")
        return losses, stats, preds, accu
    check(L.gpn_point_losses_fwd(ptr(logits), ptr(labels), ptr(offsets), ptr(gt_offsets), ptr(instance_labels), i64(M),
                                 i32(C), i64(ignore_index), ptr(losses), ptr(stats), ptr(ws), szt(ws.numel()), _stream()),
          "gpn_point_losses_fwd")
    return losses, stats


def point_losses_bwd(logits, labels, offsets, gt_offsets, instance_labels, ignore_index, stats, grad_losses):
    dev = _dev(logits, offsets)
    M, C = logits.shape
    d_logits = torch.empty((M, C), dtype=torch.float32, device=dev)
    d_offsets = torch.empty((M, 3), dtype=torch.float32, device=dev)
    check(_C.lib().gpn_point_losses_bwd(ptr(logits), ptr(labels), ptr(offsets), ptr(gt_offsets), ptr(instance_labels),
                                        i64(M), i32(C), i64(ignore_index), ptr(stats), ptr(_c(grad_losses, torch.float32)),
                                        ptr(d_logits), ptr(d_offsets), _stream()), "gpn_point_losses_bwd")
    return d_logits, d_offsets


def _p(t):
    return None if t is None else t.data_ptr()


def bn_fwd(x, res, weight, bias, running_mean, running_var, training, momentum, eps, relu):
    if not x.is_cuda:
        _dev(x)
    N, C = x.shape
    y = torch.empty_like(x)
    L = _C.lib()
    if training:
        stats = torch.empty((2, C), dtype=torch.float32, device=x.device)
        mean, invstd = stats[0], stats[1]
        ws_ptr, ws_size, stream = _fast_ws(x.device, 0)
        rc = L.gpn_bn_fwd_train(x.data_ptr(), _p(res), weight.data_ptr(), bias.data_ptr(), N, C, eps, momentum,
                                1 if relu else 0, y.data_ptr(), mean.data_ptr(), invstd.data_ptr(), _p(running_mean),
                                _p(running_var), ws_ptr, ws_size, stream)
        if rc:
            _raise("gpn_bn_fwd_train")
    else:
        mean = running_mean
        invstd = 1.0 / torch.sqrt(running_var + eps)
        rc = L.gpn_bn_fwd_eval(x.data_ptr(), _p(res), weight.data_ptr(), bias.data_ptr(), mean.data_ptr(),
                               invstd.data_ptr(), N, C, 1 if relu else 0, y.data_ptr(),
                               torch._C._cuda_getCurrentRawStream(x.device.index))
        if rc:
            _raise("gpn_bn_fwd_eval")
    return y, mean, invstd


def bn_bwd(x, y, dy, weight, mean, invstd, relu, training, has_res):
    if not x.is_cuda:
        _dev(x)
    N, C = x.shape
    dx = torch.empty_like(x)
    dres = torch.empty_like(x) if has_res else None
    dwb = torch.empty((2, C), dtype=torch.float32, device=x.device)
    dw, db = dwb[0], dwb[1]
    ws_ptr, ws_size, stream = _fast_ws(x.device, 0)
    rc = _C.lib().gpn_bn_bwd(x.data_ptr(), y.data_ptr(), dy.data_ptr(), weight.data_ptr(), mean.data_ptr(),
                             invstd.data_ptr(), N, C, 1 if relu else 0, 1 if training else 0, dx.data_ptr(), _p(dres),
                             dw.data_ptr(), db.data_ptr(), ws_ptr, ws_size, stream)
    if rc:
        _raise("gpn_bn_bwd")
    return dx, dres, dw, db


def gather_rows(table, idx, rows: Optional[DevCount] = None):
    dev = _dev(table, idx)
    table, idx = _c(table, torch.float32), _c(idx, torch.int32)
    out = torch.empty((idx.shape[0], table.shape[1]), dtype=torch.float32, device=dev)
    if rows is not None:
        check(_C.lib().gpn_gather_rows_dev(ptr(table), ptr(idx), i64(idx.shape[0]), *rows.args(), i32(table.shape[1]), ptr(out),
                                           _stream()), "gpn_gather_rows_dev")
        return out
    check(_C.lib().gpn_gather_rows(ptr(table), ptr(idx), i64(idx.shape[0]), i32(table.shape[1]), ptr(out), _stream()),
          "gpn_gather_rows")
    return out


def rows_csr(idx, n_rows):
    idx = idx.to(torch.int64)
    key = torch.where(idx >= 0, idx, torch.full_like(idx, n_rows))
    _, order = torch.sort(key, stable=True)
    counts = torch.bincount(key, minlength=n_rows + 1)[:n_rows]
    starts = torch.zeros((n_rows + 1,), dtype=torch.int32, device=idx.device)
    starts[1:] = counts.cumsum(0).to(torch.int32)
    return order.to(torch.int32), starts


def scatter_rows(dout, idx, n_rows, csr=None, rows: Optional[DevCount] = None):
    dev = _dev(dout, idx)
    dout = _c(dout, torch.float32)
    order, starts = csr if csr is not None else rows_csr(idx, n_rows)
    out = torch.empty((n_rows, dout.shape[1]), dtype=torch.float32, device=dev)
    if rows is not None:
        assert csr is not None, "a device-counted scatter needs the caller's CSR"
        check(_C.lib().gpn_scatter_rows_csr_dev(ptr(dout), ptr(_c(order, torch.int32)), ptr(_c(starts, torch.int32)), i64(n_rows),
                                                *rows.args(), i32(dout.shape[1]), ptr(out), _stream()), "gpn_scatter_rows_csr_dev")
        return out
    check(_C.lib().gpn_scatter_rows_csr(ptr(dout), ptr(_c(order, torch.int32)), ptr(_c(starts, torch.int32)),
                                        i64(n_rows), i32(dout.shape[1]), ptr(out), _stream()),
          "gpn_scatter_rows_csr")
    return out


def ball_query(points, query, batch_indices, batch_offsets, radius, num_samples, point_labels=None,
               query_labels=None):
    dev = _dev(points, query)
    points, query = _c(points, torch.float32), _c(query, torch.float32)
    bi, bo = _c(batch_indices, torch.int32), _c(batch_offsets, torch.int32)
    pl, ql = _c(point_labels, torch.int32), _c(query_labels, torch.int32)
    Q, K = query.shape[0], int(num_samples)
    idx = torch.empty((Q, K), dtype=torch.int32, device=dev)
    cnt = torch.zeros((Q,), dtype=torch.int32, device=dev)
    L = _C.lib()
    Np = points.shape[0]
    if Np >= 2048 and radius > 0:
        ws = _ws(L.gpn_ball_query_grid_ws_bytes(i64(Np)), dev)
        check(L.gpn_ball_query_grid(ptr(points), ptr(query), ptr(bi), ptr(bo), ptr(pl), ptr(ql), i64(Np), i64(Q),
                                    i64(bo.shape[0] - 1), f32(radius), i32(K), ptr(idx), ptr(cnt), ptr(ws),
                                    szt(ws.numel()), _stream()), "gpn_ball_query_grid")
        return idx, cnt
    check(L.gpn_ball_query(ptr(points), ptr(query), ptr(bi), ptr(bo), ptr(pl), ptr(ql), i64(Np),
                           i64(Q), i64(bo.shape[0] - 1), f32(radius), i32(K), ptr(idx), ptr(cnt), _stream()),
          "gpn_ball_query")
    return idx, cnt


def ccl(begin_end, edges, compacted=False):
    dev = _dev(begin_end, edges)
    be, edges = _c(begin_end, torch.int32), _c(edges, torch.int32)
    Q = be.shape[0] // 2
    labels = torch.empty((Q,), dtype=torch.int32, device=dev)
    L = _C.lib()
    ws = _ws(L.gpn_ccl_ws_bytes(i64(Q)), dev)
    check(L.gpn_ccl(ptr(be), ptr(edges), i64(Q), i64(edges.shape[0]), i32(1 if compacted else 0), ptr(labels),
                    ptr(ws), szt(ws.numel()), _stream()), "gpn_ccl")
    return labels


_MODES = {"sum": 0, "min": 1, "max": 2}


def segmented_reduce(values, begin, end, mode):
    dev = _dev(values, begin, end)
    values, begin, end = _c(values, torch.float32), _c(begin, torch.int32), _c(end, torch.int32)
    P, C = begin.shape[0], values.shape[1]
    out = torch.empty((P, C), dtype=torch.float32, device=dev)
    check(_C.lib().gpn_segmented_reduce(ptr(values), ptr(begin), ptr(end), i64(P), i32(C), i32(_MODES[mode]), ptr(out),
                                        _stream()), "gpn_segmented_reduce")
    return out


def segmented_maxpool_fwd(values, begin, end, rows: Optional[DevCount] = None):
    dev = _dev(values, begin, end)
    values, begin, end = _c(values, torch.float32), _c(begin, torch.int32), _c(end, torch.int32)
    P, C = begin.shape[0], values.shape[1]
    pooled = torch.empty((P, C), dtype=torch.float32, device=dev)
    arg = torch.empty((P, C), dtype=torch.int32, device=dev)
    if rows is not None:
        check(_C.lib().gpn_segmented_maxpool_fwd_dev(ptr(values), ptr(begin), ptr(end), i64(P), *rows.args(), i32(C), ptr(pooled),
                                                     ptr(arg), _stream()), "gpn_segmented_maxpool_fwd_dev")
        return pooled, arg
    check(_C.lib().gpn_segmented_maxpool_fwd(ptr(values), ptr(begin), ptr(end), i64(P), i32(C), ptr(pooled), ptr(arg),
                                             _stream()), "gpn_segmented_maxpool_fwd")
    return pooled, arg


def segmented_maxpool_bwd(dpooled, argmax, M, rows: Optional[DevCount] = None, m_rows: Optional[DevCount] = None):
    dev = _dev(dpooled, argmax)
    dpooled, argmax = _c(dpooled, torch.float32), _c(argmax, torch.int32)
    P, C = dpooled.shape
    dv = torch.empty((M, C), dtype=torch.float32, device=dev)
    if rows is not None:
        check(_C.lib().gpn_segmented_maxpool_bwd_dev(ptr(dpooled), ptr(argmax), i64(P), *rows.args(), i32(C), i64(M), *m_rows.args(),
                                                     ptr(dv), _stream()), "gpn_segmented_maxpool_bwd_dev")
        return dv
    check(_C.lib().gpn_segmented_maxpool_bwd(ptr(dpooled), ptr(argmax), i64(P), i32(C), i64(M), ptr(dv), _stream()),
          "gpn_segmented_maxpool_bwd")
    return dv


def instance_iou(proposal_offsets, instance_labels, batch_indices, num_points_per_instance, rows: Optional[DevCount] = None):
    dev = _dev(proposal_offsets, instance_labels, batch_indices, num_points_per_instance)
    po, il = _c(proposal_offsets, torch.int32), _c(instance_labels, torch.int32)
    bi, npi = _c(batch_indices, torch.int32), _c(num_points_per_instance, torch.int32)
    P, (B, I) = po.shape[0] - 1, npi.shape
    if rows is not None:
        out = torch.empty((P, I), dtype=torch.float32, device=dev)
        check(_C.lib().gpn_instance_iou_dev(ptr(po), ptr(il), ptr(bi), ptr(npi), i64(P), *rows.args(), i64(B), i32(I), ptr(out),
                                            _stream()), "gpn_instance_iou_dev")
        return out
    out = torch.zeros((P, I), dtype=torch.float32, device=dev)
    check(_C.lib().gpn_instance_iou(ptr(po), ptr(il), ptr(bi), ptr(npi), i64(P), i64(B), i32(I), ptr(out), _stream()),
          "gpn_instance_iou")
    return out


def nms(ious, scores, threshold):
    dev = _dev(ious, scores)
    ious, scores = _c(ious, torch.float32), _c(scores, torch.float32)
    P = scores.shape[0]
    order = torch.sort(scores, descending=True, stable=True)[1].to(torch.int32)
    keep = torch.empty((max(P, 1),), dtype=torch.int32, device=dev)
    nk = torch.zeros((1,), dtype=torch.int32, device=dev)
    L = _C.lib()
    ws = _ws(L.gpn_nms_ws_bytes(i64(P)), dev)
    check(L.gpn_nms(ptr(ious), ptr(order), i64(P), f32(threshold), ptr(keep), ptr(nk), ptr(ws), szt(ws.numel()),
                    _stream()), "gpn_nms")
    return keep[: int(nk.item())].to(torch.int64)


def pn2_ball_query(radius, nsample, xyz, new_xyz):
    dev = _dev(xyz, new_xyz)
    xyz, new_xyz = _c(xyz, torch.float32), _c(new_xyz, torch.float32)
    b, n, _ = xyz.shape
    m = new_xyz.shape[1]
    idx = torch.zeros((b, m, nsample), dtype=torch.int32, device=dev)
    check(_C.lib().gpn_pn2_ball_query(i32(b), i32(n), i32(m), f32(radius), i32(nsample), ptr(new_xyz), ptr(xyz),
                                      ptr(idx), _stream()), "gpn_pn2_ball_query")
    return idx


def pn2_group_points(points, idx):
    dev = _dev(points, idx)
    points, idx = _c(points, torch.float32), _c(idx, torch.int32)
    b, c, n = points.shape
    _, npts, ns = idx.shape
    out = torch.empty((b, c, npts, ns), dtype=torch.float32, device=dev)
    check(_C.lib().gpn_pn2_group_points(i32(b), i32(c), i32(n), i32(npts), i32(ns), ptr(points), ptr(idx), ptr(out),
                                        _stream()), "gpn_pn2_group_points")
    return out


def pn2_group_points_grad(grad_out, idx, n):
    dev = _dev(grad_out, idx)
    grad_out, idx = _c(grad_out, torch.float32), _c(idx, torch.int32)
    b, c, npts, ns = grad_out.shape
    gp = torch.zeros((b, c, n), dtype=torch.float32, device=dev)
    check(_C.lib().gpn_pn2_group_points_grad(i32(b), i32(c), i32(n), i32(npts), i32(ns), ptr(grad_out), ptr(idx),
                                             ptr(gp), _stream()), "gpn_pn2_group_points_grad")
    return gp


def pn2_gather_points(points, idx):
    dev = _dev(points, idx)
    points, idx = _c(points, torch.float32), _c(idx, torch.int32)
    b, c, n = points.shape
    m = idx.shape[1]
    out = torch.empty((b, c, m), dtype=torch.float32, device=dev)
    check(_C.lib().gpn_pn2_gather_points(i32(b), i32(c), i32(n), i32(m), ptr(points), ptr(idx), ptr(out), _stream()),
          "gpn_pn2_gather_points")
    return out


def pn2_gather_points_grad(grad_out, idx, n):
    dev = _dev(grad_out, idx)
    grad_out, idx = _c(grad_out, torch.float32), _c(idx, torch.int32)
    b, c, m = grad_out.shape
    gp = torch.zeros((b, c, n), dtype=torch.float32, device=dev)
    check(_C.lib().gpn_pn2_gather_points_grad(i32(b), i32(c), i32(n), i32(m), ptr(grad_out), ptr(idx), ptr(gp),
                                              _stream()), "gpn_pn2_gather_points_grad")
    return gp


def pn2_furthest_point_sampling(xyz, npoint):
    dev = _dev(xyz)
    xyz = _c(xyz, torch.float32)
    b, n, _ = xyz.shape
    temp = torch.full((b, n), 1e10, dtype=torch.float32, device=dev)
    idx = torch.zeros((b, npoint), dtype=torch.int32, device=dev)
    L = _C.lib()
    ws = _ws(L.gpn_pn2_furthest_point_sampling_ws_bytes(i32(b), i32(n)), dev)
    check(L.gpn_pn2_furthest_point_sampling_ws(i32(b), i32(n), i32(npoint), ptr(xyz), ptr(temp), ptr(idx), ptr(ws),
                                               szt(ws.numel()), _stream()), "gpn_pn2_furthest_point_sampling_ws")
    return idx


def pn2_three_nn(unknown, known):
    dev = _dev(unknown, known)
    unknown, known = _c(unknown, torch.float32), _c(known, torch.float32)
    b, n, _ = unknown.shape
    m = known.shape[1]
    d2 = torch.empty((b, n, 3), dtype=torch.float32, device=dev)
    idx = torch.empty((b, n, 3), dtype=torch.int32, device=dev)
    check(_C.lib().gpn_pn2_three_nn(i32(b), i32(n), i32(m), ptr(unknown), ptr(known), ptr(d2), ptr(idx), _stream()),
          "gpn_pn2_three_nn")
    return d2, idx


# ... 635 lines not shown
```

include/gpn.h:

```cpp
#ifndef GPN_H
#define GPN_H

#include <stddef.h>
#include <stdint.h>

#ifdef __cplusplus
extern "C" {
#endif

typedef void* gpn_stream_t;

#define GPN_OK 0
#define GPN_ERR_ARG 1
#define GPN_ERR_WS 2
#define GPN_ERR_HIP 3

const char* gpn_last_error(void);
int gpn_version(void);
int gpn_num_entry_points(void);
const char* gpn_entry_point_name(int i);

int gpn_linear_supported(int cin, int cout);
int gpn_linear_fwd(const float* x, const float* W, const float* b, int64_t N, int cin, int cout, float* y, gpn_stream_t stream);
size_t gpn_linear_bwd_ws_bytes(int64_t N, int cin, int cout);
// ... 81 lines not shown
                            int32_t* bwd_tile_off,
                            int64_t* num_pairs, void* ws, size_t ws_bytes, gpn_stream_t stream);

#define GPN_PACK_TRANSPOSE 1
#define GPN_PACK_REVERSE 2
#define GPN_LAYOUT_OKI 4
int gpn_spconv_pack_weights(const float* W, int K, int cin_w, int cout_w, int flags, float* packed,
                            gpn_stream_t stream);
size_t gpn_spconv_fwd_ws_bytes(int K, int64_t n_dst, int cin, int cout);
int gpn_spconv_fwd(const float* in, const float* packed_w, const int32_t* nbr, int K, int64_t n_dst, int cin,
                   int cout, float* out, void* ws, size_t ws_bytes, gpn_stream_t stream);
int gpn_spconv_fwd_ordered(const float* in, const float* packed_w, const int32_t* nbr, const int32_t* nbr_p,
                           const int32_t* perm, int K, int64_t n_dst, int cin, int cout, float* out, void* ws,
                           size_t ws_bytes, gpn_stream_t stream);
int64_t gpn_spconv_tiles_min_tiles(int64_t min_tiles);
int gpn_spconv_direct_split(int64_t split4_below_units, int64_t split2_below_units);
int gpn_spconv_msplit(int mode, int force_nt, int force_sp);
size_t gpn_spconv_fwd_w_ws_bytes(int K, int64_t n_dst, int cin, int cout);
int gpn_spconv_fwd_w(const float* in, const float* W, int K, int cin_w, int cout_w, int pack_flags, const int32_t* nbr,
                     int64_t n_dst, float* out, void* ws, size_t ws_bytes, gpn_stream_t stream);
size_t gpn_spconv_wgrad_ws_bytes(int K, int cin, int cout, int64_t n_dst);
int gpn_spconv_wgrad(const float* in, const float* dout, const int32_t* pair_src,
                     const int32_t* pair_dst, const int32_t* tile_off, int K, int64_t n_dst, int cin,
                     int cout, int flags , float* dW, void* ws,
                     size_t ws_bytes, gpn_stream_t stream);

size_t gpn_bn_ws_bytes(int64_t N, int C);
int gpn_bn_fwd_train(const float* x, const float* res, const float* weight, const float* bias, int64_t N, int C,
                     float eps, float momentum, int relu, float* y, float* mean, float* invstd, float* running_mean,
                     float* running_var, void* ws, size_t ws_bytes, gpn_stream_t stream);
int gpn_bn_fwd_eval(const float* x, const float* res, const float* weight, const float* bias, const float* mean,
                    const float* invstd, int64_t N, int C, int relu, float* y, gpn_stream_t stream);
int gpn_bn_bwd(const float* x, const float* y, const float* dy, const float* weight, const float* mean,
               const float* invstd, int64_t N, int C, int relu, int training, float* dx, float* dres, float* dweight,
               float* dbias, void* ws, size_t ws_bytes, gpn_stream_t stream);

int gpn_gather_rows(const float* table, const int32_t* idx, int64_t n, int C, float* out,
                    gpn_stream_t stream);
int gpn_scatter_rows_csr(const float* dout, const int32_t* order, const int32_t* starts,
                         int64_t n_rows, int C, float* dtable, gpn_stream_t stream);

typedef struct gpn_net_slot {
  float* data;
  float* grad;
  int64_t rows;
  int32_t channels;
  int32_t grad_state;
  const int64_t* rows_dev;
  int64_t rows_plan;
} gpn_net_slot_t;
typedef struct gpn_net_rulebook {
  const int32_t* nbr;
  const int32_t* nbr_t;
  const int32_t* nbr_p;
  const int32_t* perm;
  const int32_t* nbr_t_p;
  const int32_t* perm_t;
  const int32_t* pair_src;
  const int32_t* pair_dst;
  const int32_t* tile_off;
  int64_t n_src;
  int64_t n_dst;
  int32_t K;
  int32_t reverse_taps;
} gpn_net_rulebook_t;
typedef struct gpn_net_conv {
  const float* W;
  float* dW;
  int32_t cin;
  int32_t cout;
} gpn_net_conv_t;
typedef struct gpn_net_bn {
  const float* weight;
  const float* bias;
  float* running_mean;
  float* running_var;
  float* save_mean;
  float* save_invstd;
  float* dweight;
  float* dbias;
  float eps;
  float momentum;
  int32_t C;
  int32_t reserved;
} gpn_net_bn_t;
#define GPN_NET_CONV 0
#define GPN_NET_BN 1
#define GPN_NET_CONCAT 2
#define GPN_NET_RELU 1
#define GPN_NET_INFERENCE 2
typedef struct gpn_net_op {
  int32_t kind;
  int32_t src0;
  int32_t src1;
  int32_t dst;
  int32_t rulebook;
  int32_t param;
  int32_t flags;
  int32_t reserved;
} gpn_net_op_t;
int gpn_net_bn_fusion(int on);
int gpn_net_wgrad_group(int layers);
size_t gpn_net_ws_bytes(const gpn_net_op_t* ops, int n_ops, const gpn_net_slot_t* slots, int n_slots,
                        const gpn_net_rulebook_t* rulebooks, const gpn_net_conv_t* convs);
int gpn_net_forward(const gpn_net_op_t* ops, int n_ops, gpn_net_slot_t* slots, int n_slots,
                    const gpn_net_rulebook_t* rulebooks, int n_rulebooks, const gpn_net_conv_t* convs, int n_convs,
                    const gpn_net_bn_t* bns, int n_bns, int training, void* ws, size_t ws_bytes, gpn_stream_t stream);
int gpn_net_backward(const gpn_net_op_t* ops, int n_ops, gpn_net_slot_t* slots, int n_slots,
                     const gpn_net_rulebook_t* rulebooks, int n_rulebooks, const gpn_net_conv_t* convs, int n_convs,
                     const gpn_net_bn_t* bns, int n_bns, int training, int need_input_grad, void* ws, size_t ws_bytes,
                     gpn_stream_t stream);
int gpn_net_forward_pair(const gpn_net_op_t* ops, int n_ops, gpn_net_slot_t* slots_a, gpn_net_slot_t* slots_b, int n_slots,
                         const gpn_net_rulebook_t* rulebooks, int n_rulebooks, const gpn_net_conv_t* convs_a,
                         const gpn_net_conv_t* convs_b, int n_convs, const gpn_net_bn_t* bns_a, const gpn_net_bn_t* bns_b,
                         int n_bns, int training, void* ws, size_t ws_bytes, gpn_stream_t stream);
int gpn_net_backward_pair(const gpn_net_op_t* ops, int n_ops, gpn_net_slot_t* slots_a, gpn_net_slot_t* slots_b, int n_slots,
                          const gpn_net_rulebook_t* rulebooks, int n_rulebooks, const gpn_net_conv_t* convs_a,
                          const gpn_net_conv_t* convs_b, int n_convs, const gpn_net_bn_t* bns_a, const gpn_net_bn_t* bns_b,
                          int n_bns, int training, int need_input_grad, void* ws, size_t ws_bytes, gpn_stream_t stream);

typedef struct gpn_conv_epilogue_bf16 {
  const float* mean;
  const float* var;
  const float* weight;
  const float* bias;
  const uint16_t* res;
  float eps;
  int32_t relu;
  int32_t out_f32;
} gpn_conv_epilogue_bf16_t;
int gpn_spconv_pack_weights_bf16(const float* W, int K, int cin_w, int cout_w, int flags, uint16_t* packed, gpn_stream_t stream);
int gpn_spconv_fwd_bf16(const uint16_t* in, const uint16_t* packed_w, const int32_t* nbr, const int32_t* nbr_p, const int32_t* perm,
                        int K, int64_t n_dst, int cin, int cout, const gpn_conv_epilogue_bf16_t* ep, void* out, gpn_stream_t stream);
int gpn_rows_to_bf16(const float* x, int64_t n, int C, uint16_t* y, gpn_stream_t stream);
int gpn_bn_act_bf16(const void* x, int x_is_f32, const uint16_t* res, const float* weight, const float* bias, const float* mean,
                    const float* var, float eps, int64_t N, int C, int relu, uint16_t* y, gpn_stream_t stream);
size_t gpn_net_forward_bf16_ws_bytes(const gpn_net_op_t* ops, int n_ops, const gpn_net_slot_t* slots, int n_slots,
                                     const gpn_net_rulebook_t* rulebooks, const gpn_net_conv_t* convs);
int gpn_net_forward_bf16(const gpn_net_op_t* ops, int n_ops, gpn_net_slot_t* slots, int n_slots,
                         const gpn_net_rulebook_t* rulebooks, int n_rulebooks, const gpn_net_conv_t* convs, int n_convs,
                         const gpn_net_bn_t* bns, int n_bns, void* ws, size_t ws_bytes, gpn_stream_t stream);

int gpn_ball_query(const float* points, const float* query, const int32_t* batch_indices,
                   const int32_t* batch_offsets, const int32_t* point_labels,
                   const int32_t* query_labels, int64_t Np, int64_t Q, int64_t S, float radius, int K,
                   int32_t* indices, int32_t* count, gpn_stream_t stream);
#define GPN_BQ_NO_PAD (1 << 30)
size_t gpn_ball_query_grid_ws_bytes(int64_t Np);
int gpn_ball_query_grid(const float* points, const float* query, const int32_t* batch_indices,
                        const int32_t* batch_offsets, const int32_t* point_labels, const int32_t* query_labels,
                        int64_t Np, int64_t Q, int64_t S, float radius, int K, int32_t* indices, int32_t* count, void* ws,
                        size_t ws_bytes, gpn_stream_t stream);

size_t gpn_ccl_ws_bytes(int64_t Q);
int gpn_ccl(const int32_t* begin_end, const int32_t* edges, int64_t Q, int64_t E, int compacted,
            int32_t* labels, void* ws, size_t ws_bytes, gpn_stream_t stream);

int gpn_segmented_reduce(const float* values, const int32_t* begin, const int32_t* end, int64_t P,
                         int C, int mode, float* out, gpn_stream_t stream);
int gpn_segmented_maxpool_fwd(const float* values, const int32_t* begin, const int32_t* end, int64_t P,
                              int C, float* pooled, int32_t* argmax, gpn_stream_t stream);
int gpn_segmented_maxpool_bwd(const float* dpooled, const int32_t* argmax, int64_t P, int C, int64_t M,
                              float* dvalues, gpn_stream_t stream);

int gpn_instance_iou(const int32_t* proposal_offsets, const int32_t* instance_labels,
                     const int32_t* batch_indices, const int32_t* num_points_per_instance, int64_t P,
                     int64_t B, int I, float* ious, gpn_stream_t stream);

size_t gpn_nms_ws_bytes(int64_t P);
int gpn_nms(const float* ious, const int32_t* order, int64_t P, float threshold, int32_t* keep,
            int32_t* num_keep, void* ws, size_t ws_bytes, gpn_stream_t stream);

int gpn_pn2_ball_query(int b, int n, int m, float radius, int nsample, const float* new_xyz,
                       const float* xyz, int32_t* idx, gpn_stream_t stream);
int gpn_pn2_group_points(int b, int c, int n, int npoints, int nsample, const float* points,
                         const int32_t* idx, float* out, gpn_stream_t stream);
int gpn_pn2_group_points_grad(int b, int c, int n, int npoints, int nsample, const float* grad_out,
                              const int32_t* idx, float* grad_points, gpn_stream_t stream);
int gpn_pn2_gather_points(int b, int c, int n, int npoints, const float* points, const int32_t* idx,
                          float* out, gpn_stream_t stream);
int gpn_pn2_gather_points_grad(int b, int c, int n, int npoints, const float* grad_out,
                               const int32_t* idx, float* grad_points, gpn_stream_t stream);
int gpn_pn2_furthest_point_sampling(int b, int n, int m, const float* dataset, float* temp,
                                    int32_t* idxs, gpn_stream_t stream);
size_t gpn_pn2_furthest_point_sampling_ws_bytes(int b, int n);
int gpn_pn2_furthest_point_sampling_ws(int b, int n, int m, const float* dataset, float* temp, int32_t* idxs,
                                       void* ws, size_t ws_bytes, gpn_stream_t stream);
int gpn_pn2_three_nn(int b, int n, int m, const float* unknown, const float* known, float* dist2,
                     int32_t* idx, gpn_stream_t stream);
int gpn_pn2_knn(int b, int n, int m, int k, const float* unknown, const float* known, float* dist2,
                int32_t* idx, gpn_stream_t stream);
int gpn_pn2_three_interpolate(int b, int c, int m, int n, const float* points, const int32_t* idx,
                              const float* weight, float* out, gpn_stream_t stream);
int gpn_pn2_three_interpolate_grad(int b, int c, int n, int m, const float* grad_out,
                                   const int32_t* idx, const float* weight, float* grad_points,
                                   gpn_stream_t stream);

size_t gpn_point_losses_ws_bytes(int64_t M);
int gpn_point_losses_fwd(const float* logits, const int64_t* labels, const float* offsets, const float* gt_offsets,
                         const int32_t* instance_labels, int64_t M, int C, int64_t ignore_index, float* losses,
                         void* stats, void* ws, size_t ws_bytes, gpn_stream_t stream);
int gpn_point_losses_fwd_metrics(const float* logits, const int64_t* labels, const float* offsets, const float* gt_offsets,
                                 const int32_t* instance_labels, int64_t M, int C, int64_t ignore_index, float* losses,
                                 int64_t* preds, float* accu, void* stats_out, void* ws, size_t ws_bytes, gpn_stream_t stream);
int gpn_point_losses_bwd(const float* logits, const int64_t* labels, const float* offsets, const float* gt_offsets,
                         const int32_t* instance_labels, int64_t M, int C, int64_t ignore_index, const void* stats,
                         const float* grad_losses, float* d_logits, float* d_offsets, gpn_stream_t stream);

int gpn_score_loss(const float* logits, int C1, const int64_t* cls_i64, const int32_t* cls_i32, const int32_t* offsets,
                   const float* ious, int I, int64_t P, float fg_thresh, float bg_thresh, float* loss, float* score_preds,
                   float* d_logits, gpn_stream_t stream);

int gpn_npcs_loss_fwd(const float* logits, int n_cls3, const float* gt_npcs, const int32_t* sem_preds,
                      const int64_t* sem_labels, const int32_t* proposal_offsets, int64_t P, const int64_t* sym_of_class,
                      const float* mats, const int32_t* type_first, const int32_t* type_count, const int32_t* type_group,
                      int n_types, float* loss, void* scratch, gpn_stream_t stream);
int gpn_npcs_loss_bwd(const float* logits, int n_cls3, const float* gt_npcs, const int32_t* sem_preds,
                      const int64_t* sem_labels, const int64_t* proposal_indices, int64_t M, int64_t P,
                      const int64_t* sym_of_class, const float* mats, const int32_t* type_first, const int32_t* type_count,
                      const int32_t* type_group, int n_types, const void* scratch, const float* grad_loss, float* d_logits,
                      gpn_stream_t stream);

int64_t gpn_proposals_max_proposals(int64_t N, int min_points);
size_t gpn_proposals_build_ws_bytes(int64_t N, int64_t B, int K1, int K2, int min_points);
int gpn_proposals_build(const float* points, int point_stride, const float* offset_preds, const int64_t* sem_preds,
                        const int32_t* instance_labels, const int32_t* batch_indices, int64_t N, int64_t B, float radius,
                        int K1, int K2, int min_points, float fullscale, float max_scale, const float* jitter,
                        int64_t* counts, uint8_t* valid_mask, int64_t* valid_indices, int64_t* sorted_indices,
                        int64_t* point_indices, int64_t* proposal_indices, int32_t* batch_indices_p, float* pt_xyz_p,
                        int32_t* sem_preds_p, int32_t* instance_labels_p, int64_t* sizes, int32_t* proposal_offsets,
                        int32_t* member_slot, int32_t* voxel_coords4, int32_t* pc_voxel_id, int32_t* point_order,
                        int32_t* voxel_point_start, void* ws, size_t ws_bytes, gpn_stream_t stream);
size_t gpn_proposals_revoxelize_ws_bytes(int64_t P_ub);
int gpn_proposals_revoxelize(const float* scaled, const int32_t* proposal_offsets, int64_t* counts, int64_t T2, int64_t P_ub,
                             float fullscale, int32_t* voxel_coords3, int32_t* voxel_seg, int32_t* pc_voxel_id,
                             int32_t* point_order, int32_t* voxel_point_start, void* ws, size_t ws_bytes, gpn_stream_t stream);
int gpn_proposals_voxel_mean(const float* feats, const int64_t* point_indices, const int32_t* point_order,
                             const int32_t* voxel_point_start, int64_t V, int C, float* out, gpn_stream_t stream);
int gpn_proposals_voxel_mean_bwd(const float* dout, const int32_t* member_slot, const int32_t* pc_voxel_id,
                                 const int32_t* voxel_point_start, int64_t N, int C, float* dfeats, gpn_stream_t stream);

int gpn_backbone_prepare_desc_words(int n_levels);
size_t gpn_backbone_prepare_arena_bytes(int64_t M, int C, int64_t S, int n_levels);
int gpn_backbone_prepare(const float* points, const float* feats, const int64_t* seg_offsets, int64_t M, int C, int64_t S,
                         const float* voxel_size_host, int n_levels, uint32_t ident_levels, int64_t tile_order_min_rows,
                         int tile_order_block, int device, void* arena, size_t arena_bytes, int64_t* desc_host,
                         int64_t* pinned_stats_host, gpn_stream_t stream);

int gpn_scene_prepare_max_instances(void);
size_t gpn_scene_prepare_ws_bytes(int B);
int gpn_scene_prepare(const float* points, const void* sem_labels, int sem_bytes, const int32_t* instance_labels,
                      const int64_t* seg_offsets, int64_t N, int C, int B, const double* mats, const double* shifts,
                      float* points_out, int32_t* batch_indices, int32_t* instance_out, float* regions,
                      int32_t* num_points_per_instance, int32_t* instance_sem_labels, int64_t* num_instances_host,
                      int32_t* overflow, void* ws, size_t ws_bytes, gpn_stream_t stream);

size_t gpn_proposals_postprocess_ws_bytes(int64_t P);
int gpn_proposals_postprocess(const float* score_preds, const int64_t* sizes, const int32_t* proposal_offsets,
                              const int64_t* point_indices, const int64_t* proposal_indices, const int32_t* member_slot, int64_t N,
                              int64_t P, const int64_t* p_dev, int64_t p_plan, float score_threshold, int64_t min_points,
                              float iou_threshold, int32_t* kept_ids, int32_t* new_offsets, int64_t* src_row, int64_t* counts,
                              void* ws, size_t ws_bytes, gpn_stream_t stream);
int64_t gpn_proposals_postprocess_lds_proposals(int64_t n);

typedef struct {
  void* param;
  const void* grad;
  void* exp_avg;
  void* exp_avg_sq;
  int64_t numel;
} gpn_adam_tensor_t;
typedef struct {
  const void* src;
  void* dst;
  int64_t numel;
} gpn_copy_seg_t;
int gpn_copy_many(const gpn_copy_seg_t* segs_host, int n_segs, gpn_stream_t stream);
int gpn_adam_blocks(int64_t numel);
int gpn_adam_step(const gpn_adam_tensor_t* table_dev, const int32_t* block_first_dev, int n_tensors, int n_blocks, double lr,
                  double beta1, double beta2, double eps, int64_t step, gpn_stream_t stream);
int gpn_adam_step_gated(const gpn_adam_tensor_t* table_dev, const int32_t* block_first_dev, int n_tensors, int n_blocks,
                        double lr, double beta1, double beta2, double eps, int64_t step, const int64_t* gate_dev,
                        int64_t* skipped_dev, gpn_stream_t stream);

#define GPN_VIEW_OK 0
#define GPN_VIEW_TOO_FEW 1
#define GPN_VIEW_LABEL_MISMATCH 2
#define GPN_VIEW_INSTANCE_BOUND 3
int gpn_view_max_instance_ids(void);
int gpn_view_backproject(const void* depth, int depth_bytes, const int32_t* sem, const int32_t* ins, const double* K, int V, int H,
                         int W, int32_t* pixel, float* points, int32_t* counts, int32_t* status, gpn_stream_t stream);
size_t gpn_view_fps_ws_bytes(int V);
int gpn_view_fps(float* points, int64_t n_bound, const int32_t* counts, int32_t* status, int V, int m, int max_groups, int32_t* idx,
                 void* ws, size_t ws_bytes, gpn_stream_t stream);
int gpn_view_finish(const void* depth, int depth_bytes, const uint8_t* rgb, const int32_t* sem, const int32_t* ins, const float* npcs,
                    const double* K, int V, int H, int W, const int32_t* pixel, const int32_t* idx, int m, int32_t* status,
                    float* xyz, float* rgb_out, int32_t* sem_out, int32_t* ins_out, float* npcs_out, int32_t* pix_out, int32_t* gt,
                    double* scale, gpn_stream_t stream);

size_t gpn_pose_fit_ws_bytes(int64_t P, int H);
int gpn_pose_fit(const double* xyz, const double* npcs, const int64_t* offsets, const int64_t* picks, int64_t P, int64_t M,
                 int H, double stop_thrsh, uint8_t* valid, double* scale, double* rotation, double* translation,
                 double* transform, double* bbox, uint8_t* inlier_mask, int64_t* best_iteration, double* residual, void* ws,
                 size_t ws_bytes, gpn_stream_t stream);

#define GPN_VISU_RGB 0
#define GPN_VISU_LABEL 1
#define GPN_VISU_LABEL_MOD20 2
#define GPN_VISU_LABEL_MOD19P1 3
// ... 74 lines not shown
```

Measured before the change: 1008.

## Run proposal ball query and CCL only over live (valid-label) points

Adds a live-list path for proposal clustering. Valid point indices are compacted into an int32 list with a device-side count, and a hashed voxel grid is built over only those points. Ball query and connected-component labelling then iterate only live queries, and ball query writes begin/end ranges directly. The goal is to skip background points and the full-size grid build. The cost is several extra kernels, hash-table atomics and a larger workspace, and the path is on by default through a global toggle.

```diff
diff --git a/gapartnet_amd/_C.py b/gapartnet_amd/_C.py
--- a/gapartnet_amd/_C.py
+++ b/gapartnet_amd/_C.py
@@ -50,6 +50,8 @@
         _lib.gpn_spconv_tiles_min_tiles.restype = i64t
         _lib.gpn_spconv_direct_split.argtypes = [i64t, i64t]
         _lib.gpn_spconv_msplit.argtypes = [i32t, i32t, i32t]
+        _lib.gpn_cluster_live.argtypes = [i32t]
+        _lib.gpn_cluster_live.restype = i32t
     return _lib
 
 
diff --git a/gapartnet_amd/csrc/ballquery.hip b/gapartnet_amd/csrc/ballquery.hip
--- a/gapartnet_amd/csrc/ballquery.hip
+++ b/gapartnet_amd/csrc/ballquery.hip
@@ -1,5 +1,7 @@
 #include "gpn_common.h"
 
+#include <algorithm>
+#include <atomic>
 #include <rocprim/rocprim.hpp>
 
 namespace {
@@ -99,6 +101,55 @@
   const float dx = __fsub_rn(qx, px), dy = __fsub_rn(qy, py), dz = __fsub_rn(qz, pz);
   const float d2 = __fadd_rn(__fadd_rn(__fmul_rn(dx, dx), __fmul_rn(dy, dy)), __fmul_rn(dz, dz));
   return d2 < r2;
+}
+
+struct QueryCtx {
+  float qx, qy, qz, r2;
+  int32_t lo, hi, ql;
+  bool use_labels;
+};
+
+__device__ __forceinline__ bool test_candidate(const QueryCtx& c, const float4* __restrict__ rec, const int32_t* __restrict__ order,
+                                               int32_t j, int32_t& o) {
+  const float4 r = rec[j];
+  if (c.use_labels && __float_as_int(r.w) != c.ql) return false;
+  if (!is_hit(c.qx, c.qy, c.qz, r.x, r.y, r.z, c.r2)) return false;
+  o = order[j];
+  return o >= c.lo && o < c.hi;
+}
+
+__device__ __forceinline__ bool append_hits(bool hit, int32_t o, uint64_t lane_lt, int32_t* __restrict__ list, int& H) {
+  const uint64_t mask = __builtin_amdgcn_ballot_w64(hit);
+  const int pos = H + __popcll(mask & lane_lt);
+  if (hit && pos < kCap) list[pos] = o;
+  H += __popcll(mask);
+  return H <= kCap;
+}
+
+__device__ __forceinline__ int write_ranked(const int32_t* __restrict__ list, int H, int K, int lane, int32_t* __restrict__ out) {
+  for (int i = lane; i < H; i += 64) {
+    const int32_t v = list[i];
+    int rank = 0;
+    for (int m = 0; m < H; ++m) rank += list[m] < v ? 1 : 0;
+    if (rank < K) out[rank] = v;
+  }
+  return H < K ? H : K;
+}
+
+__device__ __forceinline__ int scan_segment(const QueryCtx& c, const float* __restrict__ points, const int32_t* __restrict__ point_labels,
+                                            int K, int lane, uint64_t lane_lt, int32_t* __restrict__ out) {
+  int cnt = 0;
+  for (int32_t base = c.lo; base < c.hi && cnt < K; base += 64) {
+    const int32_t j = base + lane;
+    bool hit = false;
+    if (j < c.hi && (!c.use_labels || point_labels[j] == c.ql))
+      hit = is_hit(c.qx, c.qy, c.qz, points[(int64_t)j * 3], points[(int64_t)j * 3 + 1], points[(int64_t)j * 3 + 2], c.r2);
+    const uint64_t mask = __builtin_amdgcn_ballot_w64(hit);
+    const int pos = cnt + __popcll(mask & lane_lt);
+    if (hit && pos < K) out[pos] = j;
+    cnt += __popcll(mask);
+  }
+  return cnt < K ? cnt : K;
 }
 
 __global__ __launch_bounds__(kThreads) void bq_query_kernel(
@@ -122,6 +173,7 @@
   }
   int32_t* out = indices + q * K;
   const uint64_t lane_lt = (1ull << lane) - 1ull;
+  const QueryCtx ctx{qx, qy, qz, r2, lo, hi, ql, use_labels};
 
   bool fallback = hdr->overflow != 0u || b > 65535;
   int H = 0;
@@ -168,45 +220,273 @@
           if (c >= 0 && c < len[t]) j = start[t] + c;
           c -= len[t];
         }
-        const float4 r = rec[j];
-        if (!use_labels || __float_as_int(r.w) == ql) {
-          if (is_hit(qx, qy, qz, r.x, r.y, r.z, r2)) {
-            o = order[j];
-            hit = o >= lo && o < hi;
+        hit = test_candidate(ctx, rec, order, j, o);
+      }
+      if (!append_hits(hit, o, lane_lt, hits[wave], H)) fallback = true;
+    }
+  }
+  const int result = fallback ? scan_segment(ctx, points, point_labels, K, lane, lane_lt, out) : write_ranked(hits[wave], H, K, lane, out);
+  if (lane == 0) count[q] = result;
+}
+
+constexpr uint64_t kKeyTag = 1ull << 47;
+
+struct LiveHeader {
+  unsigned int inv_min[3];
+  unsigned int overflow;
+  unsigned int cursor;
+  unsigned int pad;
+  unsigned long long n_points, n_queries;
+};
+
+struct LiveGrid {
+  LiveHeader* hdr;
+  unsigned long long* keys;
+  int32_t* cnt;
+  int2* range;
+  int2* where;
+  float4* rec;
+  int32_t* order;
+  int shift;
+  unsigned int mask;
+};
+
+__device__ __forceinline__ unsigned int slot_of(uint64_t key, int shift) { return (unsigned int)((key * 0x9E3779B97F4A7C15ull) >> shift); }
+
+__global__ __launch_bounds__(kThreads) void bq_live_lists_kernel(const int32_t* __restrict__ point_labels,
+                                                                 const int32_t* __restrict__ query_labels, int64_t Np, int64_t Q,
+                                                                 LiveHeader* hdr, int32_t* __restrict__ lp, int32_t* __restrict__ lq) {
+  const int lane = threadIdx.x & 63;
+  const uint64_t lane_lt = (1ull << lane) - 1ull;
+  const int64_t total = Np + Q;
+  for (int64_t base = ((int64_t)blockIdx.x * kThreads + threadIdx.x) - lane; base < total; base += (int64_t)gridDim.x * kThreads) {
+    const int64_t i = base + lane;
+    const bool isp = lp != nullptr && i < Np && point_labels[i] >= 0;
+    const bool isq = lq != nullptr && i >= Np && i < total && query_labels[i - Np] >= 0;
+    const uint64_t mp = __builtin_amdgcn_ballot_w64(isp), mq = __builtin_amdgcn_ballot_w64(isq);
+    if (mp) {
+      unsigned long long at = 0;
+      if (lane == __builtin_ctzll(mp)) at = atomicAdd(&hdr->n_points, (unsigned long long)__popcll(mp));
+      at = __shfl(at, __builtin_ctzll(mp), 64);
+      if (isp) lp[at + __popcll(mp & lane_lt)] = (int32_t)i;
+    }
+    if (mq) {
+      unsigned long long at = 0;
+      if (lane == __builtin_ctzll(mq)) at = atomicAdd(&hdr->n_queries, (unsigned long long)__popcll(mq));
+      at = __shfl(at, __builtin_ctzll(mq), 64);
+      if (isq) lq[at + __popcll(mq & lane_lt)] = (int32_t)(i - Np);
+    }
+  }
+}
+
+__global__ __launch_bounds__(kThreads) void bq_min_live_kernel(const float* __restrict__ points, int64_t Np,
+                                                               const int32_t* __restrict__ lp, const int64_t* __restrict__ np_dev,
+                                                               LiveHeader* hdr) {
+  __shared__ unsigned int smin[3];
+  if (threadIdx.x < 3) smin[threadIdx.x] = 0xffffffffu;
+  __syncthreads();
+  const int64_t n = gpn::live_len(lp, np_dev, Np);
+  unsigned int m[3] = {0xffffffffu, 0xffffffffu, 0xffffffffu};
+  for (int64_t i = (int64_t)blockIdx.x * kThreads + threadIdx.x; i < n; i += (int64_t)gridDim.x * kThreads) {
+    const int64_t j = lp ? lp[i] : i;
+#pragma unroll
+    for (int a = 0; a < 3; ++a) {
+      const unsigned int e = enc_float(points[j * 3 + a]);
+      m[a] = e < m[a] ? e : m[a];
+    }
+  }
+#pragma unroll
+  for (int a = 0; a < 3; ++a)
+    if (m[a] != 0xffffffffu) atomicMin(&smin[a], m[a]);
+  __syncthreads();
+  if (threadIdx.x < 3 && smin[threadIdx.x] != 0xffffffffu) atomicMax(&hdr->inv_min[threadIdx.x], ~smin[threadIdx.x]);
+}
+
+__device__ __forceinline__ void live_origin(const LiveHeader* hdr, float& ox, float& oy, float& oz) {
+  ox = dec_float(~hdr->inv_min[0]), oy = dec_float(~hdr->inv_min[1]), oz = dec_float(~hdr->inv_min[2]);
+}
+
+__global__ __launch_bounds__(kThreads) void bq_insert_kernel(const float* __restrict__ points, const int32_t* __restrict__ batch_offsets,
+                                                             int64_t Np, int64_t S, float inv_cell, const int32_t* __restrict__ lp,
+                                                             const int64_t* __restrict__ np_dev, LiveGrid g) {
+  const int64_t n = gpn::live_len(lp, np_dev, Np);
+  float ox, oy, oz;
+  live_origin(g.hdr, ox, oy, oz);
+  for (int64_t i = (int64_t)blockIdx.x * kThreads + threadIdx.x; i < n; i += (int64_t)gridDim.x * kThreads) {
+    const int64_t j = lp ? lp[i] : i;
+    int64_t lo = 0, hi = S;
+    while (hi - lo > 1) {
+      const int64_t mid = (lo + hi) >> 1;
+      if ((int64_t)batch_offsets[mid] <= j) lo = mid; else hi = mid;
+    }
+    const int seg = (int)lo;
+    const int cx = cell_of(points[j * 3], ox, inv_cell), cy = cell_of(points[j * 3 + 1], oy, inv_cell),
+              cz = cell_of(points[j * 3 + 2], oz, inv_cell);
+    if (cx < 1 || cy < 1 || cz < 1 || cx > kMaxCell || cy > kMaxCell || cz > kMaxCell || seg > 65535) g.hdr->overflow = 1u;
+    const unsigned long long key = pack_key(seg & 0xffff, cx & 0x7fff, cy & 0x7fff, cz & 0x7fff) | kKeyTag;
+    unsigned int h = slot_of(key, g.shift);
+    for (;;) {
+      unsigned long long old = __hip_atomic_load(g.keys + h, __ATOMIC_RELAXED, __HIP_MEMORY_SCOPE_AGENT);
+      if (old == 0ull) old = atomicCAS(g.keys + h, 0ull, key);
+      if (old == 0ull || old == key) break;
+      h = (h + 1u) & g.mask;
+    }
+    g.where[i] = make_int2((int)h, atomicAdd(g.cnt + h, 1));
+  }
+}
+
+__global__ __launch_bounds__(kThreads) void bq_ranges_kernel(int64_t Np, const int32_t* __restrict__ lp,
+                                                             const int64_t* __restrict__ np_dev, LiveGrid g) {
+  const int64_t n = gpn::live_len(lp, np_dev, Np);
+  for (int64_t i = (int64_t)blockIdx.x * kThreads + threadIdx.x; i < n; i += (int64_t)gridDim.x * kThreads) {
+    const int2 w = g.where[i];
+    if (w.y != 0) continue;
+    const int c = g.cnt[w.x];
+    g.range[w.x] = make_int2((int)atomicAdd(&g.hdr->cursor, (unsigned int)c), c);
+  }
+}
+
+__global__ __launch_bounds__(kThreads) void bq_place_kernel(const float* __restrict__ points, const int32_t* __restrict__ point_labels,
+                                                            int64_t Np, const int32_t* __restrict__ lp,
+                                                            const int64_t* __restrict__ np_dev, LiveGrid g) {
+  const int64_t n = gpn::live_len(lp, np_dev, Np);
+  for (int64_t i = (int64_t)blockIdx.x * kThreads + threadIdx.x; i < n; i += (int64_t)gridDim.x * kThreads) {
+    const int64_t j = lp ? lp[i] : i;
+    const int2 w = g.where[i];
+    const int pos = g.range[w.x].x + w.y;
+    float4 r;
+    r.x = points[j * 3];
+    r.y = points[j * 3 + 1];
+    r.z = points[j * 3 + 2];
+    r.w = __int_as_float(point_labels ? point_labels[j] : 0);
+    g.rec[pos] = r;
+    g.order[pos] = (int32_t)j;
+  }
+}
+
+struct LiveQuery {
+  const float *points, *query;
+  const int32_t *batch_indices, *batch_offsets, *point_labels, *query_labels;
+  int64_t Np, Q;
+  float r2, inv_cell;
+  int K;
+  const int32_t* lq;
+  const int64_t* nq_dev;
+  int32_t *indices, *count, *begin_end;
+};
+
+__global__ __launch_bounds__(kThreads) void bq_query_live_kernel(LiveQuery a, LiveGrid g) {
+  __shared__ int32_t hits[kWaves][kCap];
+  const int lane = threadIdx.x & 63, wave = __builtin_amdgcn_readfirstlane(threadIdx.x >> 6);
+  const uint64_t lane_lt = (1ull << lane) - 1ull;
+  const bool use_labels = a.point_labels != nullptr && a.query_labels != nullptr;
+  const int K = a.K;
+  const int64_t nq = gpn::live_len(a.lq, a.nq_dev, a.Q);
+  const bool overflow = g.hdr->overflow != 0u;
+  float ox, oy, oz;
+  live_origin(g.hdr, ox, oy, oz);
+  for (int64_t it = (int64_t)blockIdx.x * kWaves + wave; it < nq; it += (int64_t)gridDim.x * kWaves) {
+    const int64_t q = a.lq ? (int64_t)a.lq[it] : it;
+    const int32_t ql = use_labels ? a.query_labels[q] : 0;
+    if (ql < 0) {
+      if (lane == 0) a.count[q] = 0;
+      continue;
+    }
+    const float qx = a.query[q * 3], qy = a.query[q * 3 + 1], qz = a.query[q * 3 + 2];
+    const int32_t b = a.batch_indices[q];
+    const int32_t lo = a.batch_offsets[b], hi = a.batch_offsets[b + 1];
+    int32_t* out = a.indices + q * K;
+    const QueryCtx ctx{qx, qy, qz, a.r2, lo, hi, ql, use_labels};
+
+    bool fallback = overflow || b > 65535;
+    int H = 0;
+    if (!fallback) {
+      const int cx = cell_of(qx, ox, a.inv_cell), cy = cell_of(qy, oy, a.inv_cell), cz = cell_of(qz, oz, a.inv_cell);
+      int32_t start = 0, len = 0;
+      if (lane < 27) {
+        const int x = cx + lane / 9 - 1, y = cy + (lane / 3) % 3 - 1, z = cz + lane % 3 - 1;
+        if (x >= 1 && y >= 1 && z >= 1 && x <= kMaxCell && y <= kMaxCell && z <= kMaxCell) {
+          const unsigned long long key = pack_key(b, x, y, z) | kKeyTag;
+          unsigned int h = slot_of(key, g.shift);
+          for (;;) {
+            const unsigned long long k = g.keys[h];
+            if (k == key) {
+              const int2 r = g.range[h];
+              start = r.x, len = r.y;
+              break;
+            }
+            if (k == 0ull) break;
+            h = (h + 1u) & g.mask;
           }
         }
       }
-      const uint64_t mask = __builtin_amdgcn_ballot_w64(hit);
-      const int pos = H + __popcll(mask & lane_lt);
-      if (hit && pos < kCap) hits[wave][pos] = o;
-      H += __popcll(mask);
-      if (H > kCap) fallback = true;
-    }
-  }
-
-  if (!fallback) {
-    for (int i = lane; i < H; i += 64) {
-      const int32_t v = hits[wave][i];
-      int rank = 0;
-      for (int m = 0; m < H; ++m) rank += hits[wave][m] < v ? 1 : 0;
-      if (rank < K) out[rank] = v;
-    }
-    if (lane == 0) count[q] = H < K ? H : K;
-    return;
-  }
-
-  int cnt = 0;
-  for (int32_t base = lo; base < hi && cnt < K; base += 64) {
-    const int32_t j = base + lane;
-    bool hit = false;
-    if (j < hi && (!use_labels || point_labels[j] == ql))
-      hit = is_hit(qx, qy, qz, points[(int64_t)j * 3], points[(int64_t)j * 3 + 1], points[(int64_t)j * 3 + 2], r2);
-    const uint64_t mask = __builtin_amdgcn_ballot_w64(hit);
-    const int pos = cnt + __popcll(mask & lane_lt);
-    if (hit && pos < K) out[pos] = j;
-    cnt += __popcll(mask);
-  }
-  if (lane == 0) count[q] = cnt < K ? cnt : K;
+      int32_t incl = len;
+#pragma unroll
+      for (int off = 1; off < 32; off <<= 1) {
+        const int32_t up = __shfl_up(incl, off, 64);
+        if (lane >= off) incl += up;
+      }
+      const int32_t excl = incl - len;
+      const int total = __shfl(incl, 31, 64);
+      for (int base = 0; base < total && !fallback; base += 64) {
+        const int c = base + lane;
+        int t = 0;
+#pragma unroll
+        for (int step = 16; step >= 1; step >>= 1) {
+          const int32_t e = __shfl(excl, t + step, 64);
+          if (e <= c) t += step;
+        }
+        const int32_t j = __shfl(start, t, 64) + (c - __shfl(excl, t, 64));
+        bool hit = false;
+        int32_t o = -1;
+        if (c < total) hit = test_candidate(ctx, g.rec, g.order, j, o);
+        if (!append_hits(hit, o, lane_lt, hits[wave], H)) fallback = true;
+      }
+    }
+    const int result =
+        fallback ? scan_segment(ctx, a.points, a.point_labels, K, lane, lane_lt, out) : write_ranked(hits[wave], H, K, lane, out);
+    if (lane == 0) {
+      a.count[q] = result;
+      if (a.begin_end) a.begin_end[2 * q] = (int32_t)(q * K), a.begin_end[2 * q + 1] = (int32_t)(q * K) + result;
+    }
+    __builtin_amdgcn_wave_barrier();
+  }
+}
+
+struct LiveWs {
+  LiveGrid g;
+  int32_t *lp, *lq;
+  size_t clear_bytes, list_cap, total;
+};
+
+LiveWs carve_live(void* ws, size_t ws_bytes, int64_t Np) {
+  gpn::WsCarver w(ws, ws_bytes);
+  const size_t n = (size_t)(Np > 0 ? Np : 1);
+  int log2 = 1;
+  while (((size_t)1 << log2) < 2 * n) ++log2;
+  const size_t slots = (size_t)1 << log2;
+  LiveWs o;
+  o.g.hdr = w.take<LiveHeader>(1);
+  o.g.keys = w.take<unsigned long long>(slots);
+  o.g.cnt = w.take<int32_t>(slots);
+  o.clear_bytes = w.used;
+  o.g.range = w.take<int2>(slots);
+  o.g.where = w.take<int2>(n);
+  o.g.rec = w.take<float4>(n);
+  o.g.order = w.take<int32_t>(n);
+  o.lp = w.take<int32_t>(n);
+  o.lq = w.take<int32_t>(n);
+  o.list_cap = n;
+  o.g.shift = 64 - log2;
+  o.g.mask = (unsigned int)(slots - 1);
+  o.total = w.used;
+  return o;
+}
+
+std::atomic<int> g_cluster_live{1};
+inline unsigned live_grid(int64_t items, int per_wg) {
+  const int64_t g = gpn::cdiv(items > 0 ? items : 1, per_wg);
+  return (unsigned)(g < gpn::kLiveGridCap ? g : gpn::kLiveGridCap);
 }
 
 struct BqWs {
@@ -238,13 +518,73 @@
 
 }
 
-extern "C" size_t gpn_ball_query_grid_ws_bytes(int64_t Np) { return carve(nullptr, 0, Np).total; }
+extern "C" int gpn_cluster_live(int on) {
+  return on < 0 ? g_cluster_live.load(std::memory_order_relaxed) : g_cluster_live.exchange(on ? 1 : 0, std::memory_order_relaxed);
+}
+bool gpn::cluster_live() { return g_cluster_live.load(std::memory_order_relaxed) != 0; }
+
+extern "C" size_t gpn_ball_query_grid_ws_bytes(int64_t Np) { return std::max(carve(nullptr, 0, Np).total, carve_live(nullptr, 0, Np).total); }
+
+int gpn::ball_query_live(const float* points, const float* query, const int32_t* batch_indices, const int32_t* batch_offsets,
+                         const int32_t* point_labels, const int32_t* query_labels, int64_t Np, int64_t Q, int64_t S, float radius, int K,
+                         int32_t* indices, int32_t* count, const LiveList& live_points, const LiveList& live_queries, bool zero_inactive,
+                         int32_t* begin_end, void* ws, size_t ws_bytes, hipStream_t stream) {
+  const bool pad = !(K & GPN_BQ_NO_PAD);
+  K &= ~GPN_BQ_NO_PAD;
+  GPN_CHECK_ARG(Q >= 0 && Np >= 0 && S >= 0 && K >= 1 && radius > 0.f);
+  if (Q == 0) return GPN_OK;
+  GPN_CHECK_ARG(points && query && batch_indices && batch_offsets && indices && count);
+  GPN_CHECK_ARG(Np < (int64_t)0x7fffffff && Q < (int64_t)0x7fffffff && Q * (int64_t)K < ((int64_t)1 << 40));
+  GPN_CHECK_ARG((!live_points.idx || (live_points.n_dev && point_labels)) && (!live_queries.idx || (live_queries.n_dev && query_labels)));
+  LiveWs o = carve_live(ws, ws_bytes, Np);
+  if (!ws || ws_bytes < o.total) {
+    gpn::set_error("gpn_ball_query_grid: workspace too small (%zu needed, %zu given)", o.total, ws_bytes);
+    return GPN_ERR_WS;
+  }
+  const float r2 = radius * radius;
+  const float inv_cell = 1.0f / (1.05f * radius);
+  gpn::ProfScope prof(GPN_K_BALL_QUERY, stream, 0.0, 12.0 * (double)Np + 4.0 * (double)Q * K);
+  if (pad) GPN_CHECK_HIP(hipMemsetAsync(indices, 0xff, sizeof(int32_t) * (size_t)Q * K, stream));
+  GPN_CHECK_HIP(hipMemsetAsync(o.g.hdr, 0, o.clear_bytes, stream));
+  const bool use_labels = point_labels != nullptr && query_labels != nullptr;
+  const int32_t *lp = live_points.idx, *lq = live_queries.idx;
+  const int64_t *np_dev = live_points.n_dev, *nq_dev = live_queries.n_dev;
+  const bool build_lp = !lp && point_labels != nullptr && Np > 0;
+  const bool build_lq = !lq && use_labels && (size_t)Q <= o.list_cap;
+  if (build_lp || build_lq) {
+    hipLaunchKernelGGL(bq_live_lists_kernel, dim3(live_grid((build_lp ? Np : 0) + Q, kThreads)), dim3(kThreads), 0, stream, point_labels,
+                       query_labels, build_lp ? Np : 0, build_lq ? Q : 0, o.g.hdr, build_lp ? o.lp : nullptr, build_lq ? o.lq : nullptr);
+    GPN_CHECK_LAUNCH();
+    if (build_lp) lp = o.lp, np_dev = reinterpret_cast<const int64_t*>(&o.g.hdr->n_points);
+    if (build_lq) lq = o.lq, nq_dev = reinterpret_cast<const int64_t*>(&o.g.hdr->n_queries);
+  }
+  if (lq && zero_inactive) GPN_CHECK_HIP(hipMemsetAsync(count, 0, sizeof(int32_t) * (size_t)Q, stream));
+  if (Np > 0) {
+    const unsigned pgrid = live_grid(Np, kThreads);
+    hipLaunchKernelGGL(bq_min_live_kernel, dim3(pgrid < 256 ? pgrid : 256), dim3(kThreads), 0, stream, points, Np, lp, np_dev, o.g.hdr);
+    GPN_CHECK_LAUNCH();
+    hipLaunchKernelGGL(bq_insert_kernel, dim3(pgrid), dim3(kThreads), 0, stream, points, batch_offsets, Np, S, inv_cell, lp, np_dev, o.g);
+    GPN_CHECK_LAUNCH();
+    hipLaunchKernelGGL(bq_ranges_kernel, dim3(pgrid), dim3(kThreads), 0, stream, Np, lp, np_dev, o.g);
+    GPN_CHECK_LAUNCH();
+    hipLaunchKernelGGL(bq_place_kernel, dim3(pgrid), dim3(kThreads), 0, stream, points, point_labels, Np, lp, np_dev, o.g);
+    GPN_CHECK_LAUNCH();
+  }
+  const LiveQuery a{points, query, batch_indices, batch_offsets, point_labels, query_labels, Np, Q, r2, inv_cell, K, lq, nq_dev,
+                    indices, count, begin_end};
+  hipLaunchKernelGGL(bq_query_live_kernel, dim3(live_grid(Q, kWaves)), dim3(kThreads), 0, stream, a, o.g);
+  GPN_CHECK_LAUNCH();
+  return GPN_OK;
+}
 
 extern "C" int gpn_ball_query_grid(const float* points, const float* query, const int32_t* batch_indices,
                                    const int32_t* batch_offsets, const int32_t* point_labels,
                                    const int32_t* query_labels, int64_t Np, int64_t Q, int64_t S, float radius, int K,
                                    int32_t* indices, int32_t* count, void* ws, size_t ws_bytes, gpn_stream_t stream_) {
   hipStream_t stream = (hipStream_t)stream_;
+  if (gpn::cluster_live())
+    return gpn::ball_query_live(points, query, batch_indices, batch_offsets, point_labels, query_labels, Np, Q, S, radius, K, indices,
+                                count, gpn::LiveList(), gpn::LiveList(), true, nullptr, ws, ws_bytes, stream);
   const bool pad = !(K & GPN_BQ_NO_PAD);
   K &= ~GPN_BQ_NO_PAD;
   GPN_CHECK_ARG(Q >= 0 && Np >= 0 && S >= 0 && K >= 1 && radius > 0.f);
diff --git a/gapartnet_amd/csrc/cluster.hip b/gapartnet_amd/csrc/cluster.hip
--- a/gapartnet_amd/csrc/cluster.hip
+++ b/gapartnet_amd/csrc/cluster.hip
@@ -109,11 +109,8 @@
   if (r != (int32_t)i) __hip_atomic_store(parent + i, r, __ATOMIC_RELAXED, __HIP_MEMORY_SCOPE_WORKGROUP);
 }
 
-__global__ void ccl_hook_kernel(const int32_t* __restrict__ begin_end, const int32_t* __restrict__ edges,
-                                int64_t Q, int32_t* parent) {
-  const int64_t v = ((int64_t)blockIdx.x * blockDim.x + threadIdx.x) >> 6;
-  const int lane = threadIdx.x & 63;
-  if (v >= Q) return;
+__device__ __forceinline__ void ccl_hook_vertex(const int32_t* __restrict__ begin_end, const int32_t* __restrict__ edges, int64_t Q,
+                                                int32_t* parent, int64_t v, int lane) {
   const int32_t b = begin_end[2 * v], e = begin_end[2 * v + 1];
   for (int32_t t0 = b; t0 < e; t0 += 64) {
     const int32_t t = t0 + lane;
@@ -139,6 +136,14 @@
   }
 }
 
+__global__ void ccl_hook_kernel(const int32_t* __restrict__ begin_end, const int32_t* __restrict__ edges,
+                                int64_t Q, int32_t* parent) {
+  const int64_t v = ((int64_t)blockIdx.x * blockDim.x + threadIdx.x) >> 6;
+  const int lane = threadIdx.x & 63;
+  if (v >= Q) return;
+  ccl_hook_vertex(begin_end, edges, Q, parent, v, lane);
+}
+
 __global__ void ccl_flatten_kernel(int32_t* parent, int64_t Q, int32_t* __restrict__ labels,
                                    int32_t* __restrict__ is_root) {
   int64_t i = (int64_t)blockIdx.x * blockDim.x + threadIdx.x;
@@ -146,6 +151,42 @@
   const int32_t r = uf_find(parent, (int32_t)i);
   labels[i] = r;
   if (is_root) is_root[i] = (r == (int32_t)i) ? 1 : 0;
+}
+
+__global__ void ccl_self_kernel(int32_t* __restrict__ parent, int64_t Q) {
+  const int64_t i = (int64_t)blockIdx.x * blockDim.x + threadIdx.x;
+  if (i < Q) parent[i] = (int32_t)i;
+}
+
+__global__ __launch_bounds__(kThreads) void ccl_init_live_kernel(const int32_t* __restrict__ begin_end, const int32_t* __restrict__ edges,
+                                                                 int64_t Q, const int32_t* __restrict__ live,
+                                                                 const int64_t* __restrict__ n_dev, int32_t* parent) {
+  const int lane = threadIdx.x & 63, wave = __builtin_amdgcn_readfirstlane(threadIdx.x >> 6);
+  const int64_t n = gpn::live_len(live, n_dev, Q);
+  for (int64_t it = (int64_t)blockIdx.x * (kThreads / 64) + wave; it < n; it += (int64_t)gridDim.x * (kThreads / 64)) {
+    const int64_t v = live ? (int64_t)live[it] : it;
+    const int32_t b = begin_end[2 * v], e = begin_end[2 * v + 1];
+    int32_t m = (int32_t)v;
+    for (int32_t t = b + lane; t < e; t += 64) {
+      const int32_t u = edges[t];
+      if (u >= 0 && u < m) m = u;
+    }
+#pragma unroll
+    for (int off = 32; off >= 1; off >>= 1) {
+      const int32_t o = __shfl_xor(m, off, 64);
+      m = o < m ? o : m;
+    }
+    if (lane == 0) parent[v] = m;
+  }
+}
+
+__global__ __launch_bounds__(kThreads) void ccl_hook_live_kernel(const int32_t* __restrict__ begin_end, const int32_t* __restrict__ edges,
+                                                                 int64_t Q, const int32_t* __restrict__ live,
+                                                                 const int64_t* __restrict__ n_dev, int32_t* parent) {
+  const int lane = threadIdx.x & 63, wave = __builtin_amdgcn_readfirstlane(threadIdx.x >> 6);
+  const int64_t n = gpn::live_len(live, n_dev, Q);
+  for (int64_t it = (int64_t)blockIdx.x * (kThreads / 64) + wave; it < n; it += (int64_t)gridDim.x * (kThreads / 64))
+    ccl_hook_vertex(begin_end, edges, Q, parent, live ? (int64_t)live[it] : it, lane);
 }
 
 __global__ void ccl_rank_kernel(const int32_t* __restrict__ is_root, int64_t Q, int32_t* __restrict__ rank) {
@@ -384,6 +425,38 @@
   return GPN_OK;
 }
 
+int gpn::ccl_live(const int32_t* begin_end, const int32_t* edges, int64_t Q, int64_t E, const LiveList& live, int32_t* labels, void* ws,
+                  size_t ws_bytes, hipStream_t stream) {
+  GPN_CHECK_ARG(Q >= 0 && E >= 0);
+  if (Q == 0) return GPN_OK;
+  GPN_CHECK_ARG(begin_end && labels && (edges || E == 0) && (!live.idx || live.n_dev));
+  GPN_CHECK_ARG(Q < (int64_t)0x7fffffff / 64);
+  gpn::WsCarver w(ws, ws_bytes);
+  int32_t* parent = w.take<int32_t>((size_t)Q);
+  GPN_CHECK_WS(w);
+  const int grid = (int)gpn::cdiv(Q, kThreads);
+  const int64_t wgrid = gpn::cdiv(Q, kThreads / 64);
+  const dim3 lgrid((unsigned)(wgrid < gpn::kLiveGridCap ? wgrid : gpn::kLiveGridCap));
+  gpn::ProfScope prof(GPN_K_CCL, stream, 0.0, 4.0 * ((double)E + 2.0 * (double)Q) + 4.0 * (double)Q);
+  if (live.idx) {
+    hipLaunchKernelGGL(ccl_self_kernel, dim3(grid), dim3(kThreads), 0, stream, parent, Q);
+    GPN_CHECK_LAUNCH();
+  }
+  hipLaunchKernelGGL(ccl_init_live_kernel, lgrid, dim3(kThreads), 0, stream, begin_end, edges, Q, live.idx, live.n_dev, parent);
+  GPN_CHECK_LAUNCH();
+  hipLaunchKernelGGL(ccl_compress_kernel, dim3(grid), dim3(kThreads), 0, stream, parent, Q);
+  GPN_CHECK_LAUNCH();
+  hipLaunchKernelGGL(ccl_hook_live_kernel, lgrid, dim3(kThreads), 0, stream, begin_end, edges, Q, live.idx, live.n_dev, parent);
+  GPN_CHECK_LAUNCH();
+  hipLaunchKernelGGL(ccl_flatten_kernel, dim3(grid), dim3(kThreads), 0, stream, parent, Q, labels, (int32_t*)nullptr);
+  GPN_CHECK_LAUNCH();
+  return GPN_OK;
+}
+extern "C" int gpn_ccl_live(const int32_t* begin_end, const int32_t* edges, int64_t Q, int64_t E, const int32_t* live,
+                            const int64_t* n_live, int32_t* labels, void* ws, size_t ws_bytes, gpn_stream_t stream_) {
+  return gpn::ccl_live(begin_end, edges, Q, E, gpn::LiveList{live, n_live}, labels, ws, ws_bytes, (hipStream_t)stream_);
+}
+
 extern "C" int gpn_segmented_reduce(const float* values, const int32_t* begin, const int32_t* end, int64_t P,
                                     int C, int mode, float* out, gpn_stream_t stream_) {
   hipStream_t stream = (hipStream_t)stream_;
diff --git a/gapartnet_amd/csrc/gpn_common.h b/gapartnet_amd/csrc/gpn_common.h
--- a/gapartnet_amd/csrc/gpn_common.h
+++ b/gapartnet_amd/csrc/gpn_common.h
@@ -50,6 +50,24 @@
   g = (g + mult - 1) / mult * mult;
   return (unsigned)g;
 }
+
+struct LiveList {
+  const int32_t* idx = nullptr;
+  const int64_t* n_dev = nullptr;
+};
+constexpr int kLiveGridCap = 2048;
+#ifdef __HIPCC__
+__device__ __forceinline__ int64_t live_len(const int32_t* idx, const int64_t* n_dev, int64_t bound) {
+  return idx ? live_rows(n_dev, bound) : bound;
+}
+#endif
+bool cluster_live();
+int ball_query_live(const float* points, const float* query, const int32_t* batch_indices, const int32_t* batch_offsets,
+                    const int32_t* point_labels, const int32_t* query_labels, int64_t Np, int64_t Q, int64_t S, float radius, int K,
+                    int32_t* indices, int32_t* count, const LiveList& live_points, const LiveList& live_queries, bool zero_inactive,
+                    int32_t* begin_end, void* ws, size_t ws_bytes, hipStream_t stream);
+int ccl_live(const int32_t* begin_end, const int32_t* edges, int64_t Q, int64_t E, const LiveList& live, int32_t* labels, void* ws,
+             size_t ws_bytes, hipStream_t stream);
 
 constexpr int kMaxDevices = 64;
 
diff --git a/gapartnet_amd/csrc/gpn_core.hip b/gapartnet_amd/csrc/gpn_core.hip
--- a/gapartnet_amd/csrc/gpn_core.hip
+++ b/gapartnet_amd/csrc/gpn_core.hip
@@ -31,7 +31,7 @@
     "gpn_voxelize", "gpn_voxelize_ws_bytes", "gpn_rulebook_subm3", "gpn_rulebook_subm3_ws_bytes",
     "gpn_rulebook_down", "gpn_rulebook_down_ws_bytes", "gpn_rulebook_down_lists",
     "gpn_rulebook_down_lists_ws_bytes", "gpn_rulebook_level_counts", "gpn_rulebook_identity", "gpn_rulebook_level_counts_ws_bytes", "gpn_voxelize_ex", "gpn_voxelize_scenes", "gpn_voxelize_scenes_sorted", "gpn_voxelize_scenes_ws_bytes", "gpn_spconv_pack_weights", "gpn_spconv_fwd", "gpn_spconv_fwd_ws_bytes", "gpn_spconv_fwd_ordered", "gpn_rulebook_tile_order_ws_bytes", "gpn_rulebook_tile_order", "gpn_spconv_tiles_min_tiles", "gpn_spconv_direct_split", "gpn_spconv_msplit", "gpn_spconv_fwd_w", "gpn_spconv_fwd_w_ws_bytes", "gpn_spconv_wgrad",
-    "gpn_spconv_wgrad_ws_bytes", "gpn_gather_rows", "gpn_scatter_rows_csr", "gpn_bn_ws_bytes", "gpn_bn_fwd_train", "gpn_bn_fwd_eval", "gpn_bn_bwd", "gpn_net_ws_bytes", "gpn_net_bn_fusion", "gpn_net_wgrad_group", "gpn_net_forward", "gpn_linear_supported", "gpn_linear_fwd", "gpn_linear_bwd_ws_bytes", "gpn_linear_bwd", "gpn_net_backward", "gpn_net_forward_pair", "gpn_net_backward_pair", "gpn_point_losses_ws_bytes", "gpn_point_losses_fwd", "gpn_point_losses_fwd_metrics", "gpn_point_losses_bwd", "gpn_score_loss", "gpn_npcs_loss_fwd", "gpn_npcs_loss_bwd", "gpn_ball_query", "gpn_ball_query_grid_ws_bytes", "gpn_ball_query_grid", "gpn_ccl",
+    "gpn_spconv_wgrad_ws_bytes", "gpn_gather_rows", "gpn_scatter_rows_csr", "gpn_bn_ws_bytes", "gpn_bn_fwd_train", "gpn_bn_fwd_eval", "gpn_bn_bwd", "gpn_net_ws_bytes", "gpn_net_bn_fusion", "gpn_net_wgrad_group", "gpn_net_forward", "gpn_linear_supported", "gpn_linear_fwd", "gpn_linear_bwd_ws_bytes", "gpn_linear_bwd", "gpn_net_backward", "gpn_net_forward_pair", "gpn_net_backward_pair", "gpn_point_losses_ws_bytes", "gpn_point_losses_fwd", "gpn_point_losses_fwd_metrics", "gpn_point_losses_bwd", "gpn_score_loss", "gpn_npcs_loss_fwd", "gpn_npcs_loss_bwd", "gpn_ball_query", "gpn_ball_query_grid_ws_bytes", "gpn_ball_query_grid", "gpn_cluster_live", "gpn_ccl", "gpn_ccl_live",
     "gpn_ccl_ws_bytes", "gpn_segmented_reduce", "gpn_segmented_maxpool_fwd", "gpn_segmented_maxpool_bwd",
     "gpn_instance_iou", "gpn_nms", "gpn_nms_ws_bytes", "gpn_pn2_ball_query", "gpn_pn2_group_points",
     "gpn_pn2_group_points_grad", "gpn_pn2_gather_points", "gpn_pn2_gather_points_grad",
diff --git a/gapartnet_amd/csrc/proposals.hip b/gapartnet_amd/csrc/proposals.hip
--- a/gapartnet_amd/csrc/proposals.hip
+++ b/gapartnet_amd/csrc/proposals.hip
@@ -33,10 +33,11 @@
 
 __global__ __launch_bounds__(kThreads) void prop_valid_kernel(const int32_t* __restrict__ flag,
                                                               const int32_t* __restrict__ rank, int64_t N,
-                                                              int64_t* __restrict__ valid_indices, int64_t* __restrict__ counts) {
+                                                              int64_t* __restrict__ valid_indices, int32_t* __restrict__ valid32,
+                                                              int64_t* __restrict__ counts) {
   const int64_t i = (int64_t)blockIdx.x * kThreads + threadIdx.x;
   if (i >= N) return;
-  if (flag[i]) valid_indices[rank[i]] = i;
+  if (flag[i]) valid_indices[rank[i]] = i, valid32[rank[i]] = (int32_t)i;
   if (i == N - 1) counts[kQ] = (int64_t)rank[i] + flag[i];
 }
 
@@ -534,7 +535,7 @@
 }
 
 struct PropWs {
-  int32_t *lab, *flag, *rank, *scene_off, *cnt, *begin_end, *la, *lb, *start, *incl, *run_pos, *run_size, *keep_run, *new_pid,
+  int32_t *lab, *flag, *rank, *valid32, *scene_off, *cnt, *begin_end, *la, *lb, *start, *incl, *run_pos, *run_size, *keep_run, *new_pid,
       *keep_elem, *slot, *vc3, *vseg, *nbr, *rv_nvox, *rv_nout, *rv_vbase, *rv_kbase, *rv_obase;
   uint32_t *keys, *skeys, *vals, *svals;
   float *xyz, *xyz_shift, *mean, *scale, *shift, *scaled, *rmin, *rmax, *vf;
@@ -560,6 +561,7 @@
   const size_t n = (size_t)(N > 0 ? N : 1), t2 = 2 * n, pu = (size_t)P_ub + 1;
   PropWs o;
   o.lab = w.take<int32_t>(n), o.flag = w.take<int32_t>(n), o.rank = w.take<int32_t>(n);
+  o.valid32 = w.take<int32_t>(n);
   o.scene_off = w.take<int32_t>((size_t)B + 2);
   o.cnt = w.take<int32_t>(n), o.begin_end = w.take<int32_t>(2 * n), o.la = w.take<int32_t>(n), o.lb = w.take<int32_t>(n);
   o.start = w.take<int32_t>(t2), o.incl = w.take<int32_t>(t2), o.run_pos = w.take<int32_t>(t2), o.run_size = w.take<int32_t>(t2);
@@ -647,7 +649,7 @@
   GPN_CHECK_LAUNCH();
   size_t tmp = o.prim_bytes;
   GPN_CHECK_HIP(rocprim::exclusive_scan(o.prim, tmp, o.flag, o.rank, 0, (size_t)N, rocprim::plus<int32_t>(), stream));
-  hipLaunchKernelGGL(prop_valid_kernel, dim3(grid_of(N)), dim3(kThreads), 0, stream, o.flag, o.rank, N, valid_indices, counts);
+  hipLaunchKernelGGL(prop_valid_kernel, dim3(grid_of(N)), dim3(kThreads), 0, stream, o.flag, o.rank, N, valid_indices, o.valid32, counts);
   GPN_CHECK_LAUNCH();
   hipLaunchKernelGGL(prop_scene_offsets_kernel, dim3((int)gpn::cdiv(B + 1, 64)), dim3(64), 0, stream, batch_indices, N, B,
                      o.scene_off);
@@ -656,11 +658,21 @@
   const float* coords[2] = {o.xyz, o.xyz_shift};
   const int ks[2] = {K1, K2};
   int32_t* labels[2] = {o.la, o.lb};
+  const bool live = gpn::cluster_live();
+  const gpn::LiveList valid{o.valid32, counts + kQ};
   for (int set = 0; set < 2; ++set) {
     hipStream_t st = stream;
     int32_t *nbr = o.nbr, *cnt = o.cnt, *begin_end = o.begin_end;
     void* sub = o.sub;
     const size_t sub_bytes = o.sub_bytes;
+    if (live) {
+      int rc = gpn::ball_query_live(coords[set], coords[set], batch_indices, o.scene_off, o.lab, o.lab, N, N, B, radius,
+                                    ks[set] | GPN_BQ_NO_PAD, nbr, cnt, valid, valid, false, begin_end, sub, sub_bytes, st);
+      if (rc) return rc;
+      rc = gpn::ccl_live(begin_end, nbr, N, N * (int64_t)ks[set], valid, labels[set], sub, sub_bytes, st);
+      if (rc) return rc;
+      continue;
+    }
     int rc = gpn_ball_query_grid(coords[set], coords[set], batch_indices, o.scene_off, o.lab, o.lab, N, N, B, radius,
                                  ks[set] | GPN_BQ_NO_PAD, nbr, cnt, sub, sub_bytes, (gpn_stream_t)st);
     if (rc) return rc;
diff --git a/gapartnet_amd/hip_ops.py b/gapartnet_amd/hip_ops.py
--- a/gapartnet_amd/hip_ops.py
+++ b/gapartnet_amd/hip_ops.py
@@ -715,6 +715,20 @@
     ws = _ws(L.gpn_ccl_ws_bytes(i64(Q)), dev)
     check(L.gpn_ccl(ptr(be), ptr(edges), i64(Q), i64(edges.shape[0]), i32(1 if compacted else 0), ptr(labels),
                     ptr(ws), szt(ws.numel()), _stream()), "gpn_ccl")
+    return labels
+
+
+def ccl_live(begin_end, edges, live, n_live):
+    dev = _dev(begin_end, edges)
+    be, edges = _c(begin_end, torch.int32), _c(edges, torch.int32)
+    live = _c(live, torch.int32)
+    assert live is None or (n_live.dtype == torch.int64 and n_live.is_cuda)
+    Q = be.shape[0] // 2
+    labels = torch.empty((Q,), dtype=torch.int32, device=dev)
+    L = _C.lib()
+    ws = _ws(L.gpn_ccl_ws_bytes(i64(Q)), dev)
+    check(L.gpn_ccl_live(ptr(be), ptr(edges), i64(Q), i64(edges.shape[0]), ptr(live), ptr(n_live if live is not None else None),
+                         ptr(labels), ptr(ws), szt(ws.numel()), _stream()), "gpn_ccl_live")
     return labels
 
 
diff --git a/include/gpn.h b/include/gpn.h
--- a/include/gpn.h
+++ b/include/gpn.h
@@ -257,9 +257,13 @@
                         int64_t Np, int64_t Q, int64_t S, float radius, int K, int32_t* indices, int32_t* count, void* ws,
                         size_t ws_bytes, gpn_stream_t stream);
 
+int gpn_cluster_live(int on);
+
 size_t gpn_ccl_ws_bytes(int64_t Q);
 int gpn_ccl(const int32_t* begin_end, const int32_t* edges, int64_t Q, int64_t E, int compacted,
             int32_t* labels, void* ws, size_t ws_bytes, gpn_stream_t stream);
+int gpn_ccl_live(const int32_t* begin_end, const int32_t* edges, int64_t Q, int64_t E, const int32_t* live, const int64_t* n_live,
+                 int32_t* labels, void* ws, size_t ws_bytes, gpn_stream_t stream);
 
 int gpn_segmented_reduce(const float* values, const int32_t* begin, const int32_t* end, int64_t P,
                          int C, int mode, float* out, gpn_stream_t stream);
```

New measurement: 974.8. -3.3%, worse.
